# stephenbeckr/SparsifiedKMeans

Measured on AMD Instinct MI355X. Metric: Lloyd iters/sec + achieved HBM GB/s, N=1e8 d=1024 K=100, higher is better.
Workload: dtype f64

## Files before the change

### include/spkm.h

```cpp
#ifndef SPKM_H
#define SPKM_H
#include <stddef.h>
#include <stdint.h>

#ifdef __cplusplus
extern "C" {
#endif

#define SPKM_OK 0
#define SPKM_ERR_NULL_ARG (-1)
#define SPKM_ERR_CENTER_ROWS (-2)
#define SPKM_ERR_BETA_K (-3)
#define SPKM_ERR_LEN_LE_1 (-4)
#define SPKM_ERR_NOT_POW2 (-5)
#define SPKM_ERR_BAD_CSC (-6)
#define SPKM_ERR_UNSUPPORTED (-7)
#define SPKM_ERR_NO_DEVICE (-8)
#define SPKM_ERR_BAD_VALUE (-9)

typedef struct spkm_ctx spkm_ctx;
typedef struct spkm_shard spkm_shard;

const char *spkm_strerror(int status);
int spkm_version(void);

int spkm_ctx_create(int device, void *stream, spkm_ctx **out);
void spkm_ctx_destroy(spkm_ctx *ctx);
int spkm_ctx_sync(spkm_ctx *ctx);
int spkm_ctx_reload_switches(spkm_ctx *ctx);
int spkm_device_info(spkm_ctx *ctx, int64_t info[4]);


int spkm_SparseMatrixMinusCluster_host(spkm_ctx *ctx, uint64_t p, uint64_t n, const uint64_t *jc,
                                       const uint64_t *ir, const double *x, uint64_t c_rows, uint64_t K,
                                       const double *C, const double *beta, double *dist);

int spkm_SparseMatrixInnerProduct_host(spkm_ctx *ctx, uint64_t p, uint64_t n, const uint64_t *jc,
                                       const uint64_t *ir, const double *x, const double *c, double *ip,
                                       double *nx2);

int spkm_SparseMatrixColumnNormSq_host(spkm_ctx *ctx, uint64_t n, const uint64_t *jc, const double *x,
                                       double *nx2);

int spkm_hadamard_host(spkm_ctx *ctx, uint64_t m, uint64_t n, const double *x, double *y);
int spkm_hadamard_pthreads_host(spkm_ctx *ctx, uint64_t m, uint64_t n, const double *x, double *y);


int spkm_shard_create_host(spkm_ctx *ctx, uint64_t p, uint64_t n, const uint64_t *jc, const uint64_t *ir,
                           const double *x, spkm_shard **out);
int spkm_shard_create_dev(spkm_ctx *ctx, uint64_t p, uint64_t n, uint64_t nnz, const int64_t *d_jc,
                          const void *d_ir, int ir_bits, const double *d_x, uint64_t capacity,
                          spkm_shard **out);
int spkm_shard_reset_policy(spkm_shard *s);
int spkm_shard_set_lazy_stats(spkm_shard *s, int on);
int spkm_shard_set_wide_screen(spkm_shard *s, int on);
int spkm_shard_set_far_screen(spkm_shard *s, int on);
int spkm_shard_set_sliced_sums(spkm_shard *s, int on);
int spkm_shard_set_wide_bounds(spkm_shard *s, int on);
int spkm_shard_set_far_bounds(spkm_shard *s, int on);
int spkm_shard_set_far_events(spkm_shard *s, int on);
int spkm_shard_set_far_ragged(spkm_shard *s, int on);
int spkm_shard_set_tile_ragged(spkm_shard *s, int on);
int spkm_shard_release_csc(spkm_ctx *ctx, spkm_shard *s);
int spkm_shard_get_column_host(spkm_ctx *ctx, const spkm_shard *s, uint64_t col, uint64_t cap, uint64_t *ir_out,
                               double *x_out, uint64_t *count);
void spkm_shard_destroy(spkm_shard *s);
int spkm_shard_info(const spkm_shard *s, uint64_t *p, uint64_t *n, uint64_t *nnz, int *ir_bits);
int spkm_shard_order_info(const spkm_shard *s, int64_t info[2]);

uint64_t spkm_reduce_len(uint64_t p, uint64_t K);

int spkm_assign_dev(spkm_ctx *ctx, const spkm_shard *s, uint64_t K, const double *d_centers, double gamma,
                    int32_t *d_assign, double *d_mind, double *d_stats, uint64_t *d_nk_u64);

int spkm_assign_sparse_centers_dev(spkm_ctx *ctx, const spkm_shard *s, uint64_t K, const double *d_centers,
                                   const uint8_t *d_mask, double gamma, int32_t *d_assign, double *d_mind,
                                   double *d_stats, uint64_t *d_nk_u64);

int spkm_accumulate_dev(spkm_ctx *ctx, const spkm_shard *s, uint64_t K, const int32_t *d_assign,
                        double *d_reduce);

int spkm_assign_accumulate_dev(spkm_ctx *ctx, const spkm_shard *s, uint64_t K, const double *d_centers,
                               double gamma, int32_t *d_assign, double *d_mind, double *d_stats,
                               uint64_t *d_nk_u64, double *d_reduce);
int spkm_distances_dev(spkm_ctx *ctx, const spkm_shard *s, uint64_t K, const double *d_centers, double gamma,
                       const int32_t *d_assign, double *d_mind);
int spkm_distances_stats_dev(spkm_ctx *ctx, const spkm_shard *s, uint64_t K, const double *d_centers, double gamma,
                             const int32_t *d_assign, double *d_mind, double *d_stats);
int spkm_last_path_info(spkm_ctx *ctx, int64_t info[2]);
int spkm_last_screen_rounds(spkm_ctx *ctx, int64_t info[2]);
int spkm_last_screen_mode(spkm_ctx *ctx, int64_t info[8]);
int spkm_last_events_form(spkm_ctx *ctx, int64_t info[2]);
int spkm_last_assign_tile(spkm_ctx *ctx, int64_t info[6]);
int spkm_last_screen_tile(spkm_ctx *ctx, int64_t info[2]);
int spkm_last_screen_points(spkm_ctx *ctx, int64_t info[2]);
int spkm_last_mover_steps(spkm_ctx *ctx, uint64_t out[3]);
int spkm_last_mover_steps2(spkm_ctx *ctx, uint64_t out[3]);

int spkm_exact_pass_points(spkm_ctx *ctx, int64_t info[2]);
int spkm_screen_work_totals(spkm_ctx *ctx, int64_t info[2]);

int spkm_kpp_update_dev(spkm_ctx *ctx, uint64_t n, const double *d_dist_new, double *d_run, int first_round,
                        double *d_cum, double *total);
int spkm_kpp_draw_dev(spkm_ctx *ctx, uint64_t n, const double *d_cum, double target, int64_t *index);

int spkm_kpp_seed_dev(spkm_ctx *ctx, const spkm_shard *s, uint64_t K, double gamma, uint32_t R, const int64_t *first,
                      const double *u, int64_t *chosen, int32_t *status, double *d_run);
int spkm_last_kpp_plan(spkm_ctx *ctx, int info[4]);

int spkm_finalize_dev(spkm_ctx *ctx, uint64_t p, uint64_t K, const double *d_reduce, double gamma,
                      double *d_centers, double *d_out);

int spkm_fwht_dev(spkm_ctx *ctx, uint64_t m, uint64_t n, const double *d_x, double *d_y);
int spkm_mix_dev(spkm_ctx *ctx, uint64_t p, uint64_t p2, uint64_t n, const double *d_x, const double *d_sign,
                 double premul, double postdiv, double *d_y);

#define SPKM_MIX_MAX_P2 (1ull << 24)
#define SPKM_MIX_SCRATCH_BYTES (256ull << 20)
int spkm_mix_sample_dev(spkm_ctx *ctx, uint64_t p, uint64_t p2, uint64_t n, const double *d_x,
                        const double *d_sign, double premul, double postdiv, uint64_t s, uint64_t seed,
                        uint64_t col0, void *d_ir_out, int ir_bits, double *d_x_out);

uint64_t spkm_record_bytes(uint64_t s, int ir_bits);
int spkm_mix_sample_rec_dev(spkm_ctx *ctx, uint64_t p, uint64_t p2, uint64_t n, const double *d_x,
                            const double *d_sign, double premul, double postdiv, uint64_t s, uint64_t seed,
                            uint64_t col0, int ir_bits, void *d_rec_out);
#define SPKM_SKETCH_NONE 0
#define SPKM_SKETCH_DCT 1
int spkm_sketch_sample_dev(spkm_ctx *ctx, int kind, uint64_t p, uint64_t n, const double *d_x, const double *d_sign,
                           double premul, uint64_t s, uint64_t seed, uint64_t col0, void *d_ir_out, int ir_bits,
                           double *d_x_out);
int spkm_sketch_sample_rec_dev(spkm_ctx *ctx, int kind, uint64_t p, uint64_t n, const double *d_x, const double *d_sign,
                               double premul, uint64_t s, uint64_t seed, uint64_t col0, int ir_bits, void *d_rec_out);
#define SPKM_DCT_MAX_P 131072
int spkm_dct_sample_dev(spkm_ctx *ctx, uint64_t p, uint64_t n, const double *d_x, const double *d_sign, double premul,
                        uint64_t s, uint64_t seed, uint64_t col0, void *d_ir_out, int ir_bits, double *d_out);
int spkm_dct_sample_rec_dev(spkm_ctx *ctx, uint64_t p, uint64_t n, const double *d_x, const double *d_sign,
                            double premul, uint64_t s, uint64_t seed, uint64_t col0, int ir_bits, void *d_rec_out);
int spkm_dct_apply_dev(spkm_ctx *ctx, uint64_t p, uint64_t nvec, const double *d_in, const double *d_sign, int inverse,
                       double *d_out);
int spkm_shard_create_rec_dev(spkm_ctx *ctx, uint64_t p, uint64_t n, uint64_t s, int ir_bits, const void *d_rec,
                              spkm_shard **out);

#define SPKM_SRC_F64 0
#define SPKM_SRC_F32 1
#define SPKM_SRC_U8 2
#define SPKM_SRC_I16 3
#define SPKM_SRC_I32 4
#define SPKM_SRC_F16 5
#define SPKM_SRC_BF16 6
#define SPKM_SRC_I8 7
#define SPKM_SRC_U16 8

int spkm_widen_f64_dev(spkm_ctx *ctx, int kind, uint64_t count, const void *d_src, double *d_dst);

int spkm_mix_sample_src_dev(spkm_ctx *ctx, uint64_t p, uint64_t p2, uint64_t n, int src_kind, const void *d_src,
                            const double *d_sign, double premul, double postdiv, uint64_t s, uint64_t seed,
                            uint64_t col0, void *d_ir_out, int ir_bits, double *d_x_out);
int spkm_mix_sample_rec_src_dev(spkm_ctx *ctx, uint64_t p, uint64_t p2, uint64_t n, int src_kind, const void *d_src,
                                const double *d_sign, double premul, double postdiv, uint64_t s, uint64_t seed,
                                uint64_t col0, int ir_bits, void *d_rec_out);

int spkm_dense_assign_dev(spkm_ctx *ctx, uint64_t p, uint64_t n, const double *d_X, uint64_t K,
                          const double *d_centers, int32_t *d_assign, double *d_dist);
int spkm_dense_accumulate_dev(spkm_ctx *ctx, uint64_t p, uint64_t n, const double *d_X, uint64_t K,
                              const int32_t *d_assign, double *d_sums, double *d_counts);

int spkm_dense_assign_src_dev(spkm_ctx *ctx, uint64_t p, uint64_t n, int src_kind, const void *d_X, uint64_t K,
                              const double *d_centers, int32_t *d_assign, double *d_dist);
int spkm_dense_accumulate_src_dev(spkm_ctx *ctx, uint64_t p, uint64_t n, int src_kind, const void *d_X, uint64_t K,
                                  const int32_t *d_assign, double *d_sums, double *d_counts);

#define SPKM_COMM_ID_BYTES 128
#define SPKM_ERR_COMM (-10)

int spkm_comm_unique_id(uint8_t id[SPKM_COMM_ID_BYTES]);
int spkm_comm_init(spkm_ctx *ctx, int nranks, int rank, const uint8_t id[SPKM_COMM_ID_BYTES]);
int spkm_comm_destroy(spkm_ctx *ctx);
int spkm_comm_info(spkm_ctx *ctx, int *nranks, int *rank);
int spkm_allreduce_f64_dev(spkm_ctx *ctx, double *d_buf, uint64_t count);
// ... 19 lines not shown
```

### sparsifiedkmeans_amd/_lib.py

```python
from __future__ import annotations

import ctypes as C
import os
import re

_HERE = os.path.dirname(os.path.abspath(__file__))
_SO = os.path.join(_HERE, "libspkm.so")
HEADER = os.path.join(os.path.dirname(_HERE), "include", "spkm.h")

OK = 0
ERR_NULL_ARG, ERR_CENTER_ROWS, ERR_BETA_K, ERR_LEN_LE_1, ERR_NOT_POW2 = -1, -2, -3, -4, -5
ERR_BAD_CSC, ERR_UNSUPPORTED, ERR_NO_DEVICE, ERR_BAD_VALUE, ERR_COMM = -6, -7, -8, -9, -10
COMM_ID_BYTES = 128


class SpkmError(RuntimeError):

    def __init__(self, status: int, where: str = ""):
        self.status = status
        msg = lib().spkm_strerror(status).decode()
        super().__init__(f"{where + ': ' if where else ''}{msg} (spkm status {status})")


def _preload_hip_runtime() -> str:
# ... 33 lines not shown
_lib = None
hip_runtime_path = None

_u64 = C.c_uint64
_vp = C.c_void_p
_dbl = C.c_double


def declared_symbols() -> list[str]:
    with open(HEADER) as f:
        txt = f.read()
    return sorted(set(re.findall(r"\b(spkm_[A-Za-z0-9_]+)\s*\(", txt)))


def lib():
    global _lib, hip_runtime_path
    if _lib is not None:
        return _lib
    if not os.path.exists(_SO):
        raise ImportError(
            f"sparsifiedkmeans_amd: {_SO} is missing -- build it with "
            "`python -c 'import __graft_entry__ as g; g.build()'` or sparsifiedkmeans_amd/csrc/build.sh. "
            "There is no CPU fallback.")
    hip_runtime_path = _preload_hip_runtime()
    L = C.CDLL(_SO)
    L.spkm_strerror.restype = C.c_char_p
    L.spkm_strerror.argtypes = [C.c_int]
    L.spkm_version.restype = C.c_int
    L.spkm_ctx_create.argtypes = [C.c_int, _vp, C.POINTER(_vp)]
    L.spkm_ctx_destroy.argtypes = [_vp]
    L.spkm_ctx_destroy.restype = None
    L.spkm_ctx_sync.argtypes = [_vp]
    L.spkm_device_info.argtypes = [_vp, C.POINTER(C.c_int64)]
    L.spkm_SparseMatrixMinusCluster_host.argtypes = [_vp, _u64, _u64, _vp, _vp, _vp, _u64, _u64, _vp, _vp, _vp]
    L.spkm_SparseMatrixInnerProduct_host.argtypes = [_vp, _u64, _u64, _vp, _vp, _vp, _vp, _vp, _vp]
    L.spkm_SparseMatrixColumnNormSq_host.argtypes = [_vp, _u64, _vp, _vp, _vp]
    L.spkm_hadamard_host.argtypes = [_vp, _u64, _u64, _vp, _vp]
    L.spkm_hadamard_pthreads_host.argtypes = [_vp, _u64, _u64, _vp, _vp]
    L.spkm_shard_create_host.argtypes = [_vp, _u64, _u64, _vp, _vp, _vp, C.POINTER(_vp)]
    L.spkm_shard_create_dev.argtypes = [_vp, _u64, _u64, _u64, _vp, _vp, C.c_int, _vp, _u64, C.POINTER(_vp)]
    L.spkm_shard_destroy.argtypes = [_vp]
    L.spkm_shard_destroy.restype = None
    L.spkm_shard_info.argtypes = [_vp, C.POINTER(_u64), C.POINTER(_u64), C.POINTER(_u64), C.POINTER(C.c_int)]
    L.spkm_shard_order_info.argtypes = [_vp, C.POINTER(C.c_int64)]
    L.spkm_reduce_len.argtypes = [_u64, _u64]
    L.spkm_reduce_len.restype = _u64
    L.spkm_assign_dev.argtypes = [_vp, _vp, _u64, _vp, _dbl, _vp, _vp, _vp, _vp]
    L.spkm_assign_sparse_centers_dev.argtypes = [_vp, _vp, _u64, _vp, _vp, _dbl, _vp, _vp, _vp, _vp]
    L.spkm_accumulate_dev.argtypes = [_vp, _vp, _u64, _vp, _vp]
    L.spkm_assign_accumulate_dev.argtypes = [_vp, _vp, _u64, _vp, _dbl, _vp, _vp, _vp, _vp, _vp]
    L.spkm_last_path_info.argtypes = [_vp, C.POINTER(C.c_int64)]
    L.spkm_finalize_dev.argtypes = [_vp, _u64, _u64, _vp, _dbl, _vp, _vp]
    L.spkm_fwht_dev.argtypes = [_vp, _u64, _u64, _vp, _vp]
    L.spkm_mix_dev.argtypes = [_vp, _u64, _u64, _u64, _vp, _vp, _dbl, _dbl, _vp]
    L.spkm_mix_sample_dev.argtypes = [_vp, _u64, _u64, _u64, _vp, _vp, _dbl, _dbl, _u64, _u64, _u64, _vp, C.c_int, _vp]
    L.spkm_record_bytes.argtypes = [_u64, C.c_int]
    L.spkm_record_bytes.restype = _u64
    L.spkm_mix_sample_rec_dev.argtypes = [_vp, _u64, _u64, _u64, _vp, _vp, _dbl, _dbl, _u64, _u64, _u64, C.c_int, _vp]
    L.spkm_mix_sample_src_dev.argtypes = [_vp, _u64, _u64, _u64, C.c_int, _vp, _vp, _dbl, _dbl, _u64, _u64, _u64, _vp, C.c_int, _vp]
    L.spkm_mix_sample_rec_src_dev.argtypes = [_vp, _u64, _u64, _u64, C.c_int, _vp, _vp, _dbl, _dbl, _u64, _u64, _u64, C.c_int, _vp]
    L.spkm_sketch_sample_dev.argtypes = [_vp, C.c_int, _u64, _u64, _vp, _vp, _dbl, _u64, _u64, _u64, _vp, C.c_int, _vp]
    L.spkm_sketch_sample_rec_dev.argtypes = [_vp, C.c_int, _u64, _u64, _vp, _vp, _dbl, _u64, _u64, _u64, C.c_int, _vp]
    L.spkm_dct_sample_dev.argtypes = [_vp, _u64, _u64, _vp, _vp, _dbl, _u64, _u64, _u64, _vp, C.c_int, _vp]
    L.spkm_dct_sample_rec_dev.argtypes = [_vp, _u64, _u64, _vp, _vp, _dbl, _u64, _u64, _u64, C.c_int, _vp]
    L.spkm_dct_apply_dev.argtypes = [_vp, _u64, _u64, _vp, _vp, C.c_int, _vp]
    L.spkm_shard_create_rec_dev.argtypes = [_vp, _u64, _u64, _u64, C.c_int, _vp, C.POINTER(_vp)]
    L.spkm_last_screen_rounds.argtypes = [_vp, C.POINTER(C.c_int64)]
    L.spkm_last_screen_mode.argtypes = [_vp, C.POINTER(C.c_int64)]
    L.spkm_last_events_form.argtypes = [_vp, C.POINTER(C.c_int64)]
    L.spkm_last_assign_tile.argtypes = [_vp, C.POINTER(C.c_int64)]
    L.spkm_shard_reset_policy.argtypes = [_vp]
    L.spkm_shard_set_wide_screen.argtypes = [_vp, C.c_int]
    L.spkm_shard_set_wide_bounds.argtypes = [_vp, C.c_int]
    L.spkm_shard_set_far_screen.argtypes = [_vp, C.c_int]
    L.spkm_shard_set_far_bounds.argtypes = [_vp, C.c_int]
    L.spkm_shard_set_far_events.argtypes = [_vp, C.c_int]
    L.spkm_shard_set_far_ragged.argtypes = [_vp, C.c_int]
    L.spkm_shard_set_tile_ragged.argtypes = [_vp, C.c_int]
    L.spkm_shard_set_sliced_sums.argtypes = [_vp, C.c_int]
    L.spkm_last_screen_tile.argtypes = [_vp, C.POINTER(C.c_int64)]
    L.spkm_last_screen_points.argtypes = [_vp, C.POINTER(C.c_int64)]
    L.spkm_last_mover_steps.argtypes = [_vp, C.POINTER(C.c_uint64)]
    L.spkm_last_mover_steps2.argtypes = [_vp, C.POINTER(C.c_uint64)]
    L.spkm_dense_assign_dev.argtypes = [_vp, _u64, _u64, _vp, _u64, _vp, _vp, _vp]
    L.spkm_dense_accumulate_dev.argtypes = [_vp, _u64, _u64, _vp, _u64, _vp, _vp, _vp]
    L.spkm_dense_assign_src_dev.argtypes = [_vp, _u64, _u64, C.c_int, _vp, _u64, _vp, _vp, _vp]
    L.spkm_dense_accumulate_src_dev.argtypes = [_vp, _u64, _u64, C.c_int, _vp, _u64, _vp, _vp, _vp]
    L.spkm_last_assign_kernel_ms.argtypes = [_vp, C.POINTER(_dbl)]
    L.spkm_timing_log.argtypes = [_vp, C.c_int]
    L.spkm_timing_read.argtypes = [_vp, C.POINTER(_dbl), C.c_int, C.POINTER(C.c_int)]
    L.spkm_debug_block_times.argtypes = [_vp, C.c_int, C.POINTER(C.c_int64), C.c_int, C.POINTER(C.c_int)]
    L.spkm_debug_shard_bounds.argtypes = [_vp, _vp, _vp, _vp, _vp]
    L.spkm_exact_pass_points.argtypes = [_vp, C.POINTER(C.c_int64)]
    L.spkm_screen_work_totals.argtypes = [_vp, C.POINTER(C.c_int64)]
    L.spkm_distances_dev.argtypes = [_vp, _vp, _u64, _vp, _dbl, _vp, _vp]
    L.spkm_distances_stats_dev.argtypes = [_vp, _vp, _u64, _vp, _dbl, _vp, _vp, _vp]
    L.spkm_shard_set_lazy_stats.argtypes = [_vp, C.c_int]
    L.spkm_shard_release_csc.argtypes = [_vp, _vp]
    L.spkm_shard_get_column_host.argtypes = [_vp, _vp, _u64, _u64, _vp, _vp, C.POINTER(C.c_uint64)]
    L.spkm_kpp_update_dev.argtypes = [_vp, _u64, _vp, _vp, C.c_int, _vp, C.POINTER(C.c_double)]
    L.spkm_kpp_draw_dev.argtypes = [_vp, _u64, _vp, C.c_double, C.POINTER(C.c_int64)]
    L.spkm_kpp_seed_dev.argtypes = [_vp, _vp, _u64, C.c_double, C.c_uint32, _vp, _vp, _vp, _vp, _vp]
    L.spkm_last_kpp_plan.argtypes = [_vp, C.POINTER(C.c_int)]
    L.spkm_ctx_reload_switches.argtypes = [_vp]
    L.spkm_widen_f64_dev.argtypes = [_vp, C.c_int, _u64, _vp, _vp]
    L.spkm_comm_unique_id.argtypes = [_vp]
    L.spkm_comm_init.argtypes = [_vp, C.c_int, C.c_int, _vp]
    L.spkm_comm_destroy.argtypes = [_vp]
    L.spkm_comm_info.argtypes = [_vp, C.POINTER(C.c_int), C.POINTER(C.c_int)]
    L.spkm_allreduce_f64_dev.argtypes = [_vp, _vp, _u64]
    L.spkm_lloyd_iter.argtypes = [_vp, _vp, _u64, _vp, _dbl, C.c_int, _vp, _vp, _vp, _vp, _vp, _vp]
    L.spkm_lloyd_iter_host.argtypes = [_vp, _vp, _u64, _vp, _dbl, C.c_int, _vp, _vp, _vp, _vp, _vp, _vp, _vp]
    L.spkm_ctx_last_error.argtypes = [_vp]
    L.spkm_ctx_last_error.restype = C.c_char_p
    _lib = L
    return L


def check(status: int, where: str = ""):
    if status != 0:
        raise SpkmError(status, where)
```

### sparsifiedkmeans_amd/csrc/api.hip

```cpp
#include "fwht.hip"
#include "sparse_ops.hip"
#include "sample.hip"

#include "api_internal.h"
#include <chrono>
#include <sched.h>
#include <time.h>

static spkm_switches read_switches()
{
    auto on = [](const char* name) { const char* v = getenv(name); return v != nullptr && *v != 0 && !(v[0] == '0' && v[1] == 0); };
    spkm_switches w;
    w.no_screen = on("SPKM_NO_SCREEN");
    w.no_prune = on("SPKM_NO_PRUNE");
    w.no_hint = on("SPKM_NO_HINT");
    w.no_bounds = on("SPKM_NO_BOUNDS");
    w.no_rec = on("SPKM_NO_REC");
    w.no_point_list = on("SPKM_NO_POINT_LIST");
    w.no_cluster_skip = on("SPKM_NO_CLUSTER_SKIP");
    w.no_late_split = on("SPKM_NO_LATE_SPLIT");
    w.no_incremental = on("SPKM_NO_INCREMENTAL");
    w.no_support_drift = on("SPKM_NO_SUPPORT_DRIFT");
    w.no_teams = on("SPKM_NO_TEAMS");
    w.no_sums_only = on("SPKM_NO_SUMS_ONLY");
    w.no_dual = on("SPKM_NO_DUAL");
    w.no_block_skip = on("SPKM_NO_BLOCK_SKIP");
    w.no_direct_events = on("SPKM_NO_DIRECT_EVENTS");
    w.no_pair_events = on("SPKM_NO_PAIR_EVENTS");
    w.force_pair_events = on("SPKM_FORCE_PAIR_EVENTS");
    w.check_assign = on("SPKM_CHECK_ASSIGN");
    w.no_regroup = on("SPKM_NO_REGROUP");
    w.force_point_list = on("SPKM_FORCE_POINT_LIST");
    w.mover_tile = on("SPKM_NO_MOVER_TILE") ? -1 : (on("SPKM_MOVER_TILE") ? 1 : 0);
    w.mover_tile2 = on("SPKM_NO_MOVER_TILE2") ? -1 : (on("SPKM_MOVER_TILE2") ? 1 : 0);
    w.wide_screen = on("SPKM_WIDE_SCREEN");
    w.wide_bounds = on("SPKM_WIDE_BOUNDS");
    w.far_screen = on("SPKM_FAR_SCREEN");
    w.far_bounds = on("SPKM_FAR_BOUNDS");
    w.far_events = on("SPKM_FAR_EVENTS");
    w.far_ragged = on("SPKM_FAR_RAGGED");
    w.tile_ragged = on("SPKM_TILE_RAGGED");
    w.sliced_sums = on("SPKM_SLICED_SUMS");
    if (const char* v = getenv("SPKM_X_SLAB_ROWS")) w.x_slab_rows = std::max(0, atoi(v));
    if (const char* v = getenv("SPKM_FORCE_FORM")) w.force_form = std::max(0, std::min(3, atoi(v)));
    if (const char* v = getenv("SPKM_X_HINT_CHUNK")) w.x_hint_chunk = atoi(v);
    if (const char* v = getenv("SPKM_X_PLAIN_CHUNK")) w.x_plain_chunk = atoi(v);
    if (const char* v = getenv("SPKM_X_CERTIFY_GRID")) w.x_certify_grid = atoi(v);
    return w;
}

hipError_t allow_lds(spkm_ctx* ctx, const void* kern, size_t bytes)
{
    static std::mutex mu;
    static std::vector<std::tuple<int, const void*, size_t>> allowed;
    std::lock_guard<std::mutex> lock(mu);
    for (auto& e : allowed)
        if (std::get<0>(e) == ctx->device && std::get<1>(e) == kern) {
            if (std::get<2>(e) >= bytes) return hipSuccess;
            hipError_t r = hipFuncSetAttribute(kern, hipFuncAttributeMaxDynamicSharedMemorySize, (int)bytes);
            if (r == hipSuccess) std::get<2>(e) = bytes;
            return r;
        }
    hipError_t r = hipFuncSetAttribute(kern, hipFuncAttributeMaxDynamicSharedMemorySize, (int)bytes);
    if (r == hipSuccess) allowed.emplace_back(ctx->device, kern, bytes);
    return r;
}

int ensure(spkm_ctx* ctx, devbuf& b, size_t bytes)
{
    if (bytes <= b.cap && b.p) return SPKM_OK;
    if (b.p) ctx->sort_owner = nullptr;
    if (b.p) HIP_TRY(hipFree(b.p));
    b.p = nullptr;
    b.cap = 0;
    const size_t want = std::max<size_t>(bytes, 256);
    HIP_TRY(hipMalloc(&b.p, want));
    b.cap = want;
    return SPKM_OK;
}
void release(devbuf& b)
{
    if (b.p) (void)hipFree(b.p);
    b.p = nullptr;
    b.cap = 0;
}

extern "C" const char* spkm_strerror(int status)
{
    switch (status) {
    case SPKM_OK: return "ok";
    case SPKM_ERR_NULL_ARG: return "required pointer argument is NULL";
    case SPKM_ERR_CENTER_ROWS: return "Center vector must be or pxk, but this vector did not have p rows";
    case SPKM_ERR_BETA_K: return "Have not yet implemented case for using 'beta' with p x k (k!=1) centers";
    case SPKM_ERR_LEN_LE_1: return "Vector length must be greater than 1.";
    case SPKM_ERR_NOT_POW2: return "Vector length must be power of 2.";
    case SPKM_ERR_BAD_CSC: return "sparse matrix is not valid CSC (jc not monotone, row index out of range, or rows not ascending)";
    case SPKM_ERR_UNSUPPORTED: return "shape not supported by this build";
    case SPKM_ERR_NO_DEVICE: return "no usable HIP device (gfx950) available";
    case SPKM_ERR_BAD_VALUE: return "scalar argument out of range";
    case SPKM_ERR_COMM: return "RCCL is not available or an RCCL call failed (see spkm_ctx_last_error)";
    default: break;
    }
    if (status > 0) return hipGetErrorString((hipError_t)status);
    return "unknown spkm status";
}

extern "C" int spkm_version(void) { return SPKM_VERSION; }

extern "C" int spkm_ctx_create(int device, void* stream, spkm_ctx** out)
{
    if (!out) return SPKM_ERR_NULL_ARG;
    *out = nullptr;
    int ndev = 0;
    if (hipGetDeviceCount(&ndev) != hipSuccess || ndev <= 0 || device < 0 || device >= ndev)
        return SPKM_ERR_NO_DEVICE;
    spkm_ctx* ctx = new spkm_ctx();
    ctx->device = device;
    ctx->sw = read_switches();
    ctx->stream = (hipStream_t)stream;
    hipError_t e = hipSetDevice(device);
    hipDeviceProp_t prop;
    if (e == hipSuccess) e = hipGetDeviceProperties(&prop, device);
    if (e != hipSuccess) { delete ctx; return (int)e; }
    ctx->num_cus = prop.multiProcessorCount;
    ctx->mem_bytes = prop.totalGlobalMem;
    int lds = 0;
    if (hipDeviceGetAttribute(&lds, hipDeviceAttributeMaxSharedMemoryPerBlock, device) != hipSuccess || lds <= 0)
        lds = (int)prop.sharedMemPerBlock;
    ctx->lds_max = (size_t)lds;
    e = hipEventCreate(&ctx->ev0);
    if (e == hipSuccess) e = hipEventCreate(&ctx->ev1);
    if (e != hipSuccess) { delete ctx; return (int)e; }
    *out = ctx;
    return SPKM_OK;
}

extern "C" void spkm_ctx_destroy(spkm_ctx* ctx)
{
    if (!ctx) return;
    (void)hipSetDevice(ctx->device);
    (void)hipStreamSynchronize(ctx->stream);
    (void)spkm_comm_destroy(ctx);
    devbuf* all[] = {&ctx->tiles, &ctx->part_acc, &ctx->part_k, &ctx->blk_obj, &ctx->blk_max, &ctx->blk_imax,
                     &ctx->nk, &ctx->stats, &ctx->perm, &ctx->offs, &ctx->cursor, &ctx->items, &ctx->nitems,
                     &ctx->bmap, &ctx->blk_dff, &ctx->ct, &ctx->tmp_assign, &ctx->tmp_mind, &ctx->mscr, &ctx->dbg, &ctx->t32, &ctx->scr_m1, &ctx->scr_m2,
                     &ctx->scr_k, &ctx->cmax, &ctx->list, &ctx->nlist, &ctx->dn_x, &ctx->dn_c, &ctx->dn_nk, &ctx->bmapq, &ctx->bmapm, &ctx->bmapm2, &ctx->todo, &ctx->todo_m, &ctx->todo_m2, &ctx->bstat, &ctx->nk_ev, &ctx->fin_ticket, &ctx->wgstat, &ctx->offs2, &ctx->cursor2, &ctx->hist2,
                     &ctx->items2, &ctx->perm_o, &ctx->mix_scr};
    for (devbuf* b : all) release(*b);
    if (ctx->h_res) (void)hipHostFree(ctx->h_res);
    for (auto& pr : ctx->tlog) { (void)hipEventDestroy(pr.first); (void)hipEventDestroy(pr.second); }
    if (ctx->ev0) (void)hipEventDestroy(ctx->ev0);
    if (ctx->ev1) (void)hipEventDestroy(ctx->ev1);
    delete ctx;
}

extern "C" int spkm_ctx_reload_switches(spkm_ctx* ctx)
{
    if (!ctx) return SPKM_ERR_NULL_ARG;
    ctx->sw = read_switches();
    return SPKM_OK;
}

extern "C" int spkm_ctx_sync(spkm_ctx* ctx)
{
    if (!ctx) return SPKM_ERR_NULL_ARG;
    HIP_TRY(hipSetDevice(ctx->device));
    HIP_TRY(hipStreamSynchronize(ctx->stream));
    return SPKM_OK;
}

extern "C" int spkm_device_info(spkm_ctx* ctx, int64_t info[4])
{
    if (!ctx || !info) return SPKM_ERR_NULL_ARG;
    info[0] = ctx->num_cus;
    info[1] = (int64_t)ctx->lds_max;
    info[2] = (int64_t)ctx->mem_bytes;
    info[3] = SPKM_WAVE;
    return SPKM_OK;
}

static int validate_csc(uint64_t p, uint64_t n, const uint64_t* jc, const uint64_t* ir)
{
    if (jc[0] != 0) return SPKM_ERR_BAD_CSC;
    for (uint64_t i = 0; i < n; i++) {
        if (jc[i + 1] < jc[i]) return SPKM_ERR_BAD_CSC;
        for (uint64_t j = jc[i]; j < jc[i + 1]; j++) {
            if (ir[j] >= p) return SPKM_ERR_BAD_CSC;
            if (j > jc[i] && ir[j] <= ir[j - 1]) return SPKM_ERR_BAD_CSC;
        }
    }
    return SPKM_OK;
}

extern "C" int spkm_shard_create_host(spkm_ctx* ctx, uint64_t p, uint64_t n, const uint64_t* jc,
                                      const uint64_t* ir, const double* x, spkm_shard** out)
{
    if (!ctx || !out || !jc || (!ir && jc[n]) || (!x && jc[n])) return SPKM_ERR_NULL_ARG;
    *out = nullptr;
    if (p == 0 || p > 0x7fffffffull || n > 0x7ff00000ull) return SPKM_ERR_UNSUPPORTED;
    int rc = validate_csc(p, n, jc, ir);
    if (rc) return rc;
    HIP_TRY(hipSetDevice(ctx->device));
    const uint64_t nnz = jc[n];
    spkm_shard* s = new spkm_shard();
    s->ctx = ctx; s->p = p; s->n = n; s->nnz = nnz; s->owned = true; s->owned_csc = true;
    s->ir_bits = (p <= 65536) ? 16 : 32;
    s->slack = 48;
    if (n > 0 && nnz > 0 && nnz % n == 0) {
        const uint64_t st = nnz / n;
        bool fixed = st <= 0x7fffffffull;
        for (uint64_t i = 0; fixed && i <= n; i++) fixed = (jc[i] == i * st);
        if (fixed) s->fixed_s = (int)st;
    }
    {
        uint64_t mx = 0;
        for (uint64_t i = 0; i < n; i++) mx = std::max(mx, jc[i + 1] - jc[i]);
        s->max_s = (int)std::min<uint64_t>(mx, 0x7fffffffull);
        s->max_s_known = true;
    }
    const size_t irb = (size_t)s->ir_bits / 8;
    hipError_t e = hipMalloc((void**)&s->jc, (n + 1) * sizeof(long long));
    if (e == hipSuccess) e = hipMalloc(&s->ir, (nnz + 48) * irb);
    if (e == hipSuccess) e = hipMalloc((void**)&s->x, (nnz + 48) * sizeof(double));
    if (e == hipSuccess) e = hipMemsetAsync(s->ir, 0, (nnz + 48) * irb, ctx->stream);
    if (e == hipSuccess) e = hipMemsetAsync(s->x, 0, (nnz + 48) * sizeof(double), ctx->stream);
    if (e != hipSuccess) { spkm_shard_destroy(s); return (int)e; }
    std::vector<long long> jcn(n + 1);
    for (uint64_t i = 0; i <= n; i++) jcn[i] = (long long)jc[i];
    e = hipMemcpyAsync(s->jc, jcn.data(), (n + 1) * sizeof(long long), hipMemcpyHostToDevice, ctx->stream);
// ... 1060 lines not shown
```

### sparsifiedkmeans_amd/csrc/api_internal.h

```cpp
#pragma once
#include <hip/hip_runtime.h>

#include "../../include/spkm.h"
#include "layout.h"
#include "policy.h"

#include <dlfcn.h>

#include <algorithm>
#include <cmath>
#include <cstdio>
#include <cstdlib>
#include <cstring>
#include <utility>
#include <mutex>
#include <tuple>
#include <vector>

#define SPKM_VERSION 100

struct devbuf {
    void* p = nullptr;
    size_t cap = 0;
};

struct spkm_switches {
    bool no_screen = false;
    bool no_prune = false;
    bool no_hint = false;
    bool no_bounds = false;
    bool no_rec = false;
    bool no_point_list = false;
    bool no_cluster_skip = false;
    int x_hint_chunk = 0;
    int x_plain_chunk = 0;
    int x_certify_grid = 0;
    bool no_late_split = false;
    bool no_incremental = false;
    bool no_support_drift = false;
    bool no_sums_only = false;
    bool no_block_skip = false;
    bool no_dual = false;
    bool no_pair_events = false;
    bool force_pair_events = false;
    bool no_direct_events = false;
    bool no_teams = false;
    bool no_regroup = false;
    bool check_assign = false;
    int force_form = 0;
    bool wide_screen = false;
    bool wide_bounds = false;
    bool far_screen = false;
    bool far_bounds = false;
    bool far_events = false;
    bool far_ragged = false;
    bool tile_ragged = false;
    bool sliced_sums = false;
    int x_slab_rows = 0;
    bool force_point_list = false;
    int mover_tile2 = 0;
    int mover_tile = 0;
};
struct spkm_screen_report {
    int path = 0;
    int kt = 0, tiles = 0;
    int pl_last = 0;
    int rounds_all = 0, rounds = 0;
    int mode = 0;
    bool hinted = false;
    bool hint_late = false;
    bool skipping = false;
    bool pt_mode = false;
    bool lib_valid = false;
    bool incremental = false;
    bool direct_events = false;
    bool pair_events = false;
    bool sums_only = false;
    bool movers2 = false;
    bool movers = false;
    bool dual = false;
};
struct spkm_ctx {
    int device = 0;
    spkm_switches sw;
    hipStream_t stream = nullptr;
    int num_cus = 0;
    size_t lds_max = 0;
    size_t mem_bytes = 0;
    devbuf tiles, part_acc, part_k, blk_obj, blk_max, blk_imax, nk, stats, perm, offs, cursor, items, nitems,
        bmap, blk_dff, ct, tmp_assign, tmp_mind, mscr, dbg, t32, scr_m1, scr_m2, scr_k, cmax, list, nlist, dn_x, dn_c, dn_nk, bmapq, bmapm, bmapm2, todo, todo_m, todo_m2, bstat, nk_ev, fin_ticket, wgstat, offs2, cursor2, hist2, items2, perm_o;
    devbuf mix_scr;
    double* h_res = nullptr;
    double* h_res_dev = nullptr;
    size_t h_res_len = 0;
    unsigned long long res_seq = 0ull;
    bool res_map_failed = false;
    int bmap_G = -1, bmap_blocks = 0, bmap_streams = 0;
    int bmapq_key = -1, bmapq_blocks = 0;
    int bmapm_key = -1, bmapm_blocks = 0;
    int bmapm2_key = -1, bmapm2_blocks = 0;
    hipEvent_t ev0 = nullptr, ev1 = nullptr;
    bool ev_valid = false;
    std::vector<std::pair<hipEvent_t, hipEvent_t>> tlog;
    size_t tlog_used = 0;
    bool tlog_on = false;
    const void* sort_owner = nullptr;
    bool sort_partial = false;
    int sort_K = 0, sort_seg = 0;
    long long sort_n = 0;
    bool tlog_both = false;
    int assign_KT = 0, assign_G = 0;
    spkm_screen_report last;
    int last_exact_pts = 0;
    int last_acc_form = 0;
    int last_dist_form = 0;
    int last_kpp[4] = {0, 0, 0, 0};
    unsigned last_listed = 0;
    bool sort_perm_valid = false;
    char errmsg[256] = {0};
    void* comm = nullptr;
    int comm_nranks = 0, comm_rank = 0;
};

struct spkm_shard {
    spkm_ctx* ctx = nullptr;
    uint64_t p = 0, n = 0, nnz = 0;
    int ir_bits = 32;
    long long* jc = nullptr;
    void* ir = nullptr;
    double* x = nullptr;
    bool owned = false;
    bool owned_csc = false;
    int fixed_s = 0;
    uint64_t slack = 0;
    bool wide = false;
    bool wide_bounds = false;
    bool far = false;
    bool far_bounds = false;
    bool far_events = false;
    bool far_ragged = false;
    bool tile_ragged = false;
    int max_s = 0;
    bool max_s_known = false;
    bool sliced = false;
    float* xfs = nullptr;
    void* irs = nullptr;
    bool norms_done = false, xf_done = false;
    float* xnr = nullptr;
    float* xf = nullptr;
    char* rec = nullptr;
    int rec_R = 0;
    bool rec_owned = true;
    bool rec_tried = false;
    unsigned* h_nlist = nullptr;
    unsigned* h_nlist_dev = nullptr;
    unsigned nlist_seq = 0;
    bool nlist_pending = false;
    spkm_policy pol;
    float* hintu = nullptr;
    long long hintu_len = 0;
    float* hb = nullptr;
    double* hb_centers = nullptr;
    size_t hb_centers_len = 0;
    long long hb_npad = 0;
    int hb_K = 0;
    double hb_gamma = 0.0;
    bool hb_valid = false;
    char* sp = nullptr;
    long long sp_blocks = 0;
    bool sp_clean = false;
    const void* sp_assign = nullptr;
    bool assign_synced = false;
    double* hb_cum = nullptr;
// ... 37 lines not shown
```

### sparsifiedkmeans_amd/csrc/api_lloyd.hip

```cpp
#include "assign.hip"
#include "update.hip"
#include "kpp.hip"
#include "screen.hip"
#include "screen_wide.hip"
#include "screen_far.hip"
#include "dense.hip"

#include "api_internal.h"

const void* spkm_sq_kernel_16_0(int rounds, int a_rounds);
const void* spkm_sq_kernel_16_1(int rounds, int a_rounds);
const void* spkm_sq_kernel_32_0(int rounds, int a_rounds);
const void* spkm_sq_kernel_32_1(int rounds, int a_rounds);
template <typename IR> static const void* screen_quad_kernel(int rounds, int a_rounds, bool pts = false)
{
    if (sizeof(IR) == 2) return pts ? spkm_sq_kernel_16_1(rounds, a_rounds) : spkm_sq_kernel_16_0(rounds, a_rounds);
    return pts ? spkm_sq_kernel_32_1(rounds, a_rounds) : spkm_sq_kernel_32_0(rounds, a_rounds);
}

extern "C" int spkm_shard_create_rec_dev(spkm_ctx* ctx, uint64_t p, uint64_t n, uint64_t s_entries, int ir_bits,
                                         const void* d_rec, spkm_shard** out)
{
    if (!ctx || !out || (n && !d_rec)) return SPKM_ERR_NULL_ARG;
    *out = nullptr;
// ... 781 lines not shown
}

extern "C" int spkm_distances_dev(spkm_ctx* ctx, const spkm_shard* s, uint64_t K64, const double* d_centers, double gamma,
                                  const int32_t* d_assign, double* d_mind)
{
    return spkm_distances_stats_dev(ctx, s, K64, d_centers, gamma, d_assign, d_mind, nullptr);
}

extern "C" int spkm_exact_pass_points(spkm_ctx* ctx, int64_t info[2])
{
    if (!ctx || !info) return SPKM_ERR_NULL_ARG;
    info[0] = info[1] = 0;
    if (ctx->nlist.p) {
        HIP_TRY(hipSetDevice(ctx->device));
        HIP_TRY(hipStreamSynchronize(ctx->stream));
        unsigned v[NL_EXACT_TOTAL + 2] = {0};
        HIP_TRY(hipMemcpy(v, ctx->nlist.p, sizeof(v), hipMemcpyDeviceToHost));
        info[0] = (int64_t)(((unsigned long long)v[NL_EXACT_TOTAL + 1] << 32) | v[NL_EXACT_TOTAL]);
        info[1] = v[NL_EXACT_PTS];
    }
    return SPKM_OK;
}

extern "C" int spkm_screen_work_totals(spkm_ctx* ctx, int64_t info[2])
{
    if (!ctx || !info) return SPKM_ERR_NULL_ARG;
    info[0] = info[1] = 0;
    if (ctx->nlist.p) {
        HIP_TRY(hipSetDevice(ctx->device));
        HIP_TRY(hipStreamSynchronize(ctx->stream));
        static_assert(NL_ROUNDS_FULL == NL_ROUNDS_DONE + 2, "the two totals are copied together");
        unsigned long long v[2] = {0ull, 0ull};
        HIP_TRY(hipMemcpy(v, (const unsigned*)ctx->nlist.p + NL_ROUNDS_DONE, sizeof(v), hipMemcpyDeviceToHost));
        info[0] = (int64_t)v[0];
        info[1] = (int64_t)v[1];
    }
    return SPKM_OK;
}

extern "C" int spkm_last_screen_points(spkm_ctx* ctx, int64_t info[2])
{
    if (!ctx || !info) return SPKM_ERR_NULL_ARG;
    info[0] = info[1] = 0;
    if (ctx->nlist.p) {
        HIP_TRY(hipSetDevice(ctx->device));
        HIP_TRY(hipStreamSynchronize(ctx->stream));
        static_assert(NL_SCREENED == NL_SCREENED_TOTAL + 2, "the total and the call's count are copied together");
        unsigned v[3] = {0u, 0u, 0u};
        HIP_TRY(hipMemcpy(v, (const unsigned*)ctx->nlist.p + NL_SCREENED_TOTAL, sizeof(v), hipMemcpyDeviceToHost));
        info[1] = (int64_t)(((unsigned long long)v[1] << 32) | v[0]);
        info[0] = ctx->last.path == 1 ? (int64_t)v[2] : 0;
    }
    return SPKM_OK;
}

extern "C" int spkm_last_mover_steps(spkm_ctx* ctx, uint64_t out[3])
{
    if (!ctx || !out) return SPKM_ERR_NULL_ARG;
    out[0] = out[1] = out[2] = 0;
    if (ctx->last.path == 1 && ctx->nlist.p) {
        HIP_TRY(hipSetDevice(ctx->device));
        HIP_TRY(hipStreamSynchronize(ctx->stream));
        unsigned v[SPKM_REPORT_WORDS] = {0};
        HIP_TRY(hipMemcpy(v, ctx->nlist.p, sizeof(v), hipMemcpyDeviceToHost));
        out[0] = v[NL_MSTEPS]; out[1] = v[NL_MCERT]; out[2] = v[NL_MSENT];
    }
    return SPKM_OK;
}

extern "C" int spkm_last_mover_steps2(spkm_ctx* ctx, uint64_t out[3])
{
    if (!ctx || !out) return SPKM_ERR_NULL_ARG;
    out[0] = out[1] = out[2] = 0;
    if (ctx->last.path == 1 && ctx->nlist.p) {
        HIP_TRY(hipSetDevice(ctx->device));
        HIP_TRY(hipStreamSynchronize(ctx->stream));
        unsigned v[SPKM_REPORT_WORDS] = {0};
        HIP_TRY(hipMemcpy(v, ctx->nlist.p, sizeof(v), hipMemcpyDeviceToHost));
        out[0] = v[NL_MSTEPS2]; out[1] = v[NL_MCERT2]; out[2] = v[NL_MSENT2];
    }
    return SPKM_OK;
}

extern "C" int spkm_last_screen_rounds(spkm_ctx* ctx, int64_t info[2])
{
    if (!ctx || !info) return SPKM_ERR_NULL_ARG;
    info[0] = ctx->last.rounds_all;
    info[1] = ctx->last.rounds;
    return SPKM_OK;
}

extern "C" int spkm_last_screen_mode(spkm_ctx* ctx, int64_t info[8])
{
    if (!ctx || !info) return SPKM_ERR_NULL_ARG;
    info[0] = -1;
    info[1] = info[2] = info[3] = info[4] = info[5] = info[6] = info[7] = 0;
    const spkm_screen_report& r = ctx->last;
    if (r.path == 1 && ctx->nlist.p) {
        HIP_TRY(hipSetDevice(ctx->device));
        HIP_TRY(hipStreamSynchronize(ctx->stream));
        unsigned v[SPKM_REPORT_WORDS] = {0};
        HIP_TRY(hipMemcpy(v, ctx->nlist.p, sizeof(v), hipMemcpyDeviceToHost));
        info[0] = r.mode;
        info[1] = v[NL_LISTED]; info[2] = v[NL_AMBIG]; info[3] = v[NL_EARLY]; info[4] = v[NL_SKIPPED];
        info[5] = (int64_t)(((unsigned long long)v[NL_SKIPPED_TOTAL + 1] << 32) | v[NL_SKIPPED_TOTAL]);
        info[6] = r.incremental ? (r.direct_events ? 4 : 2) : (r.sums_only ? 3 : 0);
        if (r.dual) info[6] = v[NL_GATE_FULL] ? 3 : 2;
        info[7] = r.pt_mode ? 2 : 0;
    }
    return SPKM_OK;
}

extern "C" int spkm_last_events_form(spkm_ctx* ctx, int64_t info[2])
{
    if (!ctx || !info) return SPKM_ERR_NULL_ARG;
    const spkm_screen_report& r = ctx->last;
    info[0] = r.incremental ? (r.direct_events ? 2 : 1) : 0;
    info[1] = (r.incremental && r.pair_events) ? 1 : 0;
    return SPKM_OK;
}

extern "C" int spkm_last_assign_tile(spkm_ctx* ctx, int64_t info[6])
{
    if (!ctx || !info) return SPKM_ERR_NULL_ARG;
    info[0] = ctx->assign_KT;
    info[1] = ctx->assign_G;
    info[2] = ctx->last.pl_last;
    info[3] = ctx->last_exact_pts;
    info[4] = ctx->last_acc_form;
    info[5] = ctx->last_dist_form;
    return SPKM_OK;
}

extern "C" int spkm_last_screen_tile(spkm_ctx* ctx, int64_t info[2])
{
    if (!ctx || !info) return SPKM_ERR_NULL_ARG;
    info[0] = ctx->last.kt;
    info[1] = ctx->last.tiles;
    return SPKM_OK;
}

extern "C" int spkm_debug_shard_bounds(spkm_ctx* ctx, const spkm_shard* s, float* ub, double* lb, int32_t* lib_assign)
{
    if (!ctx || !s) return SPKM_ERR_NULL_ARG;
    if (!s->hb || !s->hb_valid || !s->hb_cum) return SPKM_ERR_UNSUPPORTED;
    HIP_TRY(hipSetDevice(ctx->device));
    HIP_TRY(hipStreamSynchronize(ctx->stream));
    const size_t n = (size_t)s->n, npad = (size_t)s->hb_npad;
    std::vector<int> map;
    if (s->map) {
        map.resize(n);
        HIP_TRY(hipMemcpy(map.data(), s->map, n * 4, hipMemcpyDeviceToHost));
    }
    auto at = [&](size_t i) { return s->map ? (size_t)map[i] : i; };
    std::vector<float> tmp(n);
    if (ub) {
        HIP_TRY(hipMemcpy(tmp.data(), s->hb, n * 4, hipMemcpyDeviceToHost));
        for (size_t i = 0; i < n; i++) ub[at(i)] = tmp[i];
    }
    if (lib_assign) {
        std::vector<int32_t> ta(n);
        HIP_TRY(hipMemcpy(ta.data(), s->hb + hb_assign(npad), n * 4, hipMemcpyDeviceToHost));
        for (size_t i = 0; i < n; i++) lib_assign[at(i)] = ta[i];
    }
    if (lb) {
        double cum = 0.0;
// ... 356 lines not shown
```

### sparsifiedkmeans_amd/csrc/api_lloyd_fused.inc

```
static int screen_tile_kt(const spkm_ctx* ctx, const spkm_shard* s)
{
    if ((s->p + 1) * (uint64_t)SCREEN_KT * 4 + 16 <= ctx->lds_max) return SCREEN_KT;
    return (s->wide || ctx->sw.wide_screen) ? spkm_wide_kt((long long)s->p, ctx->lds_max) : 0;
}
static bool screen_use_quad(const spkm_ctx* ctx, const spkm_shard* s)
{
    return spkm_screen_quad(screen_tile_kt(ctx, s), s->fixed_s);
}
static int screen_width(const spkm_ctx* ctx, const spkm_shard* s, int K)
{
    return spkm_screen_width((long long)s->p, K, s->fixed_s, s->slack, s->nnz, ctx->lds_max, ctx->num_cus, ctx->sw.no_screen,
                             s->wide || ctx->sw.wide_screen);
}
static int far_screen_width(const spkm_ctx* ctx, const spkm_shard* s, int K)
{
    if (s->fixed_s <= 0)
        return spkm_far_screen_ragged((long long)s->p, K, s->fixed_s, s->slack, s->nnz, ctx->lds_max, ctx->num_cus, ctx->sw.no_screen,
                                      s->far || ctx->sw.far_screen, s->far_ragged || ctx->sw.far_ragged);
    return spkm_far_screen((long long)s->p, K, s->fixed_s, s->slack, s->nnz, ctx->lds_max, ctx->num_cus, ctx->sw.no_screen,
                           s->wide || ctx->sw.wide_screen, s->far || ctx->sw.far_screen);
}
static int tile_ragged_width(const spkm_ctx* ctx, const spkm_shard* s, int K)
{
    return spkm_tile_screen_ragged((long long)s->p, K, s->fixed_s, s->slack, s->nnz, ctx->lds_max, ctx->num_cus, ctx->sw.no_screen,
                                   s->tile_ragged || ctx->sw.tile_ragged);
}

static_assert(spkm_movers == SPKM_MOVERS && spkm_movers == SCREEN_KT && spkm_mover_kmin == SPKM_MOVER_KMIN && spkm_mover_kmax == SPKM_MOVER_KMAX &&
              SPKM_MOVER_KMAX <= BOUNDS_KTAB, "the mover tile is one full screen tile; policy.h and layout.h agree on its limits");
static_assert(spkm_movers2 == SPKM_MOVERS2 && spkm_movers2 == 2 * SCREEN_KT && spkm_mover2_kmin == SPKM_MOVER2_KMIN,
              "the second level is two full screen tiles; policy.h and layout.h agree on its limits");
static_assert(spkm_plan_kt == SCREEN_KT && spkm_plan_span == BOUNDS_SPAN && spkm_plan_span_pt == BOUNDS_SPAN_PT &&
              spkm_plan_seg == SEG_POINTS, "policy.h sizes the kernels with these constants");

template <typename T>
static hipError_t regrow(T*& buf, size_t bytes, bool* valid = nullptr)
{
    if (buf) (void)hipFree(buf);
    buf = nullptr;
    if (valid) *valid = false;
    const hipError_t e = hipMalloc((void**)&buf, bytes);
    if (e != hipSuccess) buf = nullptr;
    return e;
}
static int ensure_blk_stats(spkm_ctx* ctx, size_t items)
{
    int rc;
    if ((rc = ensure(ctx, ctx->blk_obj, items * 8)) || (rc = ensure(ctx, ctx->blk_max, items * 8))) return rc;
    return ensure(ctx, ctx->blk_imax, items * 8);
}
static int count_assign_diff(spkm_ctx* ctx, const spkm_shard* s, const int32_t* d_assign, long long npad, unsigned* diff)
{
    const long long n = (long long)s->n;
    unsigned* cnt = (unsigned*)ctx->nlist.p + NL_CHECK_DIFF;
    HIP_TRY(hipMemsetAsync(cnt, 0, 4, ctx->stream));
    hipLaunchKernelGGL(k_count_diff_i32, dim3((unsigned)std::min<long long>(4096, (n + 255) / 256)), dim3(256), 0, ctx->stream,
                       (const int*)d_assign, (const int*)(s->hb + hb_assign(npad)), n, cnt, (const int*)s->map);
    HIP_TRY(hipMemcpyAsync(diff, cnt, 4, hipMemcpyDeviceToHost, ctx->stream));
    HIP_TRY(hipStreamSynchronize(ctx->stream));
    return SPKM_OK;
}
struct screen_call : spkm_call_in {
    spkm_ctx* ctx;
    spkm_shard* sm;
    const double* C;
    double gamma;
    int32_t* assign;
    double *mind, *sums, *counts;
    size_t pk;
    spkm_call_plan pl;
    spkm_mover_plan mv;
    spkm_mover2_plan mv2;
    spkm_screen_report rep;
    spkm_zero_jobs zj;
    int kt = SCREEN_KT;
    bool carry = false;
    int bstat_n = 0, seg = 0, max_items = 0;
    void zero_later(void* q, size_t bytes) { zj.p[zj.n] = (unsigned*)q; zj.words[zj.n] = bytes / 4; zj.n++; }
    void zero_flush()
    {
        if (!zj.n) return;
        unsigned long long mx = 0;
        for (int q = 0; q < zj.n; q++) mx = std::max(mx, zj.words[q]);
        hipLaunchKernelGGL(k_zero_many, dim3((unsigned)std::min<unsigned long long>((mx + 1023) / 1024, 256)), dim3(256), 0,
                           ctx->stream, zj);
        zj.n = 0;
    }
    int* cl(int row) const { return pl.cl_on ? sm->cl_flags + (size_t)row * K : nullptr; }
    int col_s() const { return sm->fixed_s > 0 ? sm->fixed_s : sm->max_s; }
    bool ragged() const { return sm->fixed_s <= 0; }
    template <typename IR> int buffers()
    {
        int rc;
        if (!quad && !sm->xnr) HIP_TRY(hipMalloc((void**)&sm->xnr, (size_t)n * 4));
        if (!quad && (rc = ensure_csc(ctx, sm))) return rc;
        if (!quad && !sm->xf) {
            HIP_TRY(hipMalloc((void**)&sm->xf, (size_t)(sm->nnz + 48) * 4));
            HIP_TRY(hipMemsetAsync(sm->xf, 0, (size_t)(sm->nnz + 48) * 4, ctx->stream));
        }
        if (!quad && (!sm->norms_done || !sm->xf_done)) {
            hipLaunchKernelGGL(k_point_norms, dim3((unsigned)std::min<long long>((n + 15) / 16, 16384)), dim3(256), 0,
                               ctx->stream, (const long long*)sm->jc, (const double*)sm->x, n, sm->fixed_s, sm->xnr, sm->xf);
            sm->norms_done = sm->xf_done = true;
        }
        if (quad && !sm->xfs) {
            if (!(sm->x == nullptr && sm->rec != nullptr) && (rc = ensure_csc(ctx, sm))) return rc;
            if ((rc = build_screen_copy<IR>(ctx, sm))) return rc;
        }
        const int Gs = pl.Gs;
        if (quad) rc = build_blockmap_quad(ctx, Gs, pl.pl_last, pl.nr);
        else rc = build_blockmap(ctx, pl.G);
        if (rc) return rc;
        if ((rc = ensure(ctx, ctx->t32, (size_t)(pl.G + (quad ? 2 : 0)) * (p + 1) * kt * 4)) || (rc = ensure(ctx, ctx->cmax, 64)) ||
            (rc = ensure(ctx, ctx->scr_m1, (size_t)Gs * n * 4)) || (rc = ensure(ctx, ctx->scr_m2, (size_t)Gs * n * 4)) ||
            (rc = ensure(ctx, ctx->scr_k, (size_t)Gs * n * 4)) || (rc = ensure(ctx, ctx->list, (size_t)n * 4)))
            return rc;
        {
            const bool fresh = ctx->nlist.p == nullptr;
            if ((rc = ensure(ctx, ctx->nlist, NL_WORDS * 4))) return rc;
            if (fresh) HIP_TRY(hipMemsetAsync(ctx->nlist.p, 0, NL_WORDS * 4, ctx->stream));
        }
        if ((rc = ensure(ctx, ctx->ct, pk * 8)) || (rc = ensure(ctx, ctx->nk, (size_t)K * 8)) || (rc = ensure(ctx, ctx->stats, 4 * 8)))
            return rc;
        zero_later(ctx->cmax.p, 16);
        zero_later((unsigned*)ctx->nlist.p + NL_ZERO_A, (NL_ZERO_A_END - NL_ZERO_A) * 4);
        zero_later((unsigned*)ctx->nlist.p + NL_ZERO_B, (NL_ZERO_B_END - NL_ZERO_B) * 4);
        zero_later(sums, (2 * pk + K + 1) * 8);
        if (!carry) return SPKM_OK;
        if (!sm->hb || sm->hb_npad != pl.npad) {
            HIP_TRY(regrow(sm->hb, hb_floats(pl.npad) * 4, &sm->hb_valid));
            sm->hb_npad = pl.npad;
            HIP_TRY(hipMemsetAsync(sm->hb + hb_mticket(pl.npad), 0, (size_t)(HB_TAIL - HB_MOVERS) * 4, ctx->stream));
        }
        if (sm->hb_centers_len < pk) {
            HIP_TRY(regrow(sm->hb_centers, pk * 8, &sm->hb_valid));
            sm->hb_centers_len = pk;
        }
        bounds_valid = sm->hb_valid && sm->hb_K == K && sm->hb_gamma == gamma;
        if (!sm->hb_cum) HIP_TRY(hipMalloc((void**)&sm->hb_cum, 16));
        if (quad && sm->pol.regroup_wanted && !sm->regroup_done && bounds_valid && sm->lazy && mind == nullptr && sm->rec != nullptr &&
            sm->xfs != nullptr && !ctx->sw.no_regroup) {
            if ((rc = regroup_shard<IR>(ctx, sm, K))) return rc;
            sm->regroup_done = true;
        }
        sm->pol.regroup_wanted = false;
        if (!bounds_valid) {
            HIP_TRY(hipMemsetAsync(sm->hb_cum, 0, 16, ctx->stream));
            sm->cum_par = 0;
        }
        if (far && far_events && sm->lazy) {
            if (!sm->cl_cache || sm->cl_pk != pk || sm->cl_K != K) {
                if (regrow(sm->cl_cache, cc_doubles(pk, K) * 8, &sm->cl_valid) != hipSuccess) {
                    (void)hipGetLastError();
                    sm->cl_pk = 0; sm->cl_K = 0;
                    far_events = false;
                } else {
                    sm->cl_pk = pk; sm->cl_K = K;
                }
            }
        }
        if (!quad) return SPKM_OK;
        if (!sm->cl_cache || sm->cl_pk != pk || sm->cl_K != K) {
            HIP_TRY(regrow(sm->cl_cache, cc_doubles(pk, K) * 8, &sm->cl_valid));
            HIP_TRY(regrow(sm->cl_flags, (size_t)CL_ROWS * K * 4));
            sm->cl_pk = pk; sm->cl_K = K;
        }
        zero_later(sm->cl_flags + (size_t)CL_TOUCHED * K, (size_t)K * 4);
        return SPKM_OK;
    }
    void plan_input(int prune_a_, bool want_hint_)
    {
        const spkm_switches& sw = ctx->sw;
        teams = quad ? ctx->bmapq_blocks / 4 : ctx->bmap_streams;
        no_bounds = sw.no_bounds; no_point_list = sw.no_point_list; force_point_list = sw.force_point_list;
        no_late_split = sw.no_late_split; no_incremental = sw.no_incremental; no_pair_events = sw.no_pair_events;
        force_pair_events = sw.force_pair_events; no_block_skip = sw.no_block_skip; no_cluster_skip = sw.no_cluster_skip;
        no_sums_only = sw.no_sums_only; no_dual = sw.no_dual; no_direct_events = sw.no_direct_events;
        x_hint_chunk = sw.x_hint_chunk; x_plain_chunk = sw.x_plain_chunk;
        lazy = sm->lazy; want_dist = mind != nullptr; has_map = sm->map != nullptr;
        cl_valid = sm->cl_valid; cl_stats_valid = sm->cl_stats_valid;
        sp_clean = sm->sp_clean; sp_blocks = sm->sp_blocks;
        same_assign = sm->sp_assign == (const void*)assign; assign_synced = sm->assign_synced;
        sort_kept = ctx->sort_owner == (const void*)sm && ctx->sort_K == K && ctx->sort_n == n;
        prune_a = prune_a_; want_hint = want_hint_;
    }
    int resources()
    {
        const size_t N = (size_t)n;
        if (pl.ev_possible && sm->ev_cap < 2 * N) {
            sm->ev_cap = 0;
            if (regrow(sm->ev_pt, 2 * N * 4 + 64) != hipSuccess || regrow(sm->ev_k, 2 * N * 4 + 64) != hipSuccess) {
                (void)hipGetLastError();
                pl.lose_events();
            } else
                sm->ev_cap = 2 * N;
        }
        if (pl.pair_ev && allow_lds(ctx, (const void*)k_plan_segments_wide, (size_t)K * (size_t)(K + 1) * 4) != hipSuccess) {
            (void)hipGetLastError();
            pl.lose_pair();
        }
        if (pl.pair_ev && sm->ev_o_cap < N + 4096) {
            sm->ev_o_cap = 0;
            if (regrow(sm->ev_o, (N + 4096) * 4 + 64) != hipSuccess) {
                (void)hipGetLastError();
                pl.lose_pair();
            } else
                sm->ev_o_cap = N + 4096;
        }
        int rc;
        if (pl.ev_path) {
            if ((rc = ensure(ctx, ctx->nk_ev, (size_t)2 * K * 8))) return rc;
            zero_later(ctx->nk_ev.p, (size_t)2 * K * 8);
        }
        if (pl.hinted) {
            rep.hint_late = pl.late;
            if (sm->hintu_len < pl.npad) {
                HIP_TRY(regrow(sm->hintu, (size_t)pl.npad * 4));
                sm->hintu_len = pl.npad;
            }
        }
        return SPKM_OK;
    }
    int mover_resources()
    {
        if (!mv.on) return SPKM_OK;
        int rc;
        if ((rc = build_blockmap_quad(ctx, mv.tiles, mv.pl, mv.nr, true))) return rc;
        if ((rc = ensure(ctx, ctx->todo_m, (size_t)mv.cap * 4))) return rc;
        if (!mv2.on) return SPKM_OK;
        if ((rc = build_blockmap_quad(ctx, mv2.tiles, mv2.pl, mv2.nr, true))) return rc;
        return ensure(ctx, ctx->todo_m2, (size_t)mv2.cap * 4);
    }
    int bounds()
    {
        const long long npad = pl.npad;
        if (!carry) {
            sm->hb_valid = sm->assign_synced = false;
            return SPKM_OK;
        }
        int* same = quad ? sm->cl_flags + (size_t)CL_SAME * K : (int*)nullptr;
        if (pl.drift) {
            zero_later(sm->hb + hb_dmax(npad, K), 4);
            zero_flush();
            hipLaunchKernelGGL(k_center_drift, dim3(K), dim3(256), 0, ctx->stream, (const double*)sm->hb_centers, C, K, p,
                               gamma, sm->hb + hb_delta(npad), same, ctx->sw.no_support_drift ? 0 : col_s(),
                               2.0f * (float)sm->fixed_s / (float)p, quad ? sm->hb + hb_hterm(npad) : (float*)nullptr,
                               mv.eligible ? reinterpret_cast<unsigned*>(sm->hb + hb_mticket(npad)) : (unsigned*)nullptr,
                               sm->hb + hb_mdr(npad), reinterpret_cast<int*>(sm->hb + hb_mlist(npad)),
                               reinterpret_cast<int*>(sm->hb + hb_mslot(npad)));
            int rc;
            if ((rc = ensure(ctx, ctx->todo, pl.pt_mode ? (size_t)(npad + 64) * 4 : (size_t)(npad / 16 + 1) * 4))) return rc;
            if ((rc = ensure(ctx, ctx->bstat, (size_t)pl.bgrid * BS_STRIDE * 4))) return rc;
            const long long nblk = npad / 1024 + 1;
            if (pl.sp_on && sm->sp_blocks != nblk) {
                HIP_TRY(regrow(sm->sp, sp_bytes(nblk), &sm->sp_clean));
                sm->sp_blocks = nblk;
            }
            unsigned* sp_mask = pl.sp_on ? reinterpret_cast<unsigned*>(sm->sp) : nullptr;
            float* sp_slack = pl.sp_on ? reinterpret_cast<float*>(sm->sp + sp_off_slack(nblk)) : nullptr;
            int* sp_valid = pl.sp_on ? reinterpret_cast<int*>(sm->sp + sp_off_valid(nblk)) : nullptr;
            if (((pl.sp_on && !pl.sp_reset) || pl.trusted) && ctx->sw.check_assign) {
                unsigned diff = 0;
                if ((rc = count_assign_diff(ctx, sm, assign, npad, &diff))) return rc;
                if (diff) {
                    snprintf(ctx->errmsg, sizeof(ctx->errmsg), "SPKM_CHECK_ASSIGN: d_assign differs from the library's copy of the previous "
                             "call's assignment in %u places (lazy statistics: the buffer is the library's to keep between calls)", diff);
                    sm->sp_clean = false;
                    sm->assign_synced = false;
                    return SPKM_ERR_BAD_VALUE;
                }
            }
            const long long blocks = std::min<long long>((npad + pl.span - 1) / pl.span, pl.bgrid);
            hipLaunchKernelGGL(sm->map != nullptr ? k_bounds_steps<true> : (mv.eligible ? k_bounds_steps<false, true> : k_bounds_steps<false>),
                               dim3((unsigned)blocks), dim3(256), 0,
                               ctx->stream, sm->hb, npad, n, K, pl.trusted ? (int*)nullptr : (int*)assign, (int*)ctx->todo.p,
                               (unsigned*)ctx->nlist.p, pl.hinted ? sm->hintu : (float*)nullptr, pl.skip_enabled ? 1 : 0,
                               pl.pt_mode ? 1 : 0, (const double*)(sm->hb_cum + sm->cum_par), sm->hb_cum + (sm->cum_par ^ 1),
                               (int)pl.span, (unsigned*)ctx->bstat.p, pl.erode ? 1 : 0, sp_slack, sp_mask, sp_valid, pl.sp_reset ? 1 : 0,
                               (const int*)same, (const int*)sm->map, mv.on ? (int*)ctx->todo_m.p : (int*)nullptr,
                               mv2.on ? (int*)ctx->todo_m2.p : (int*)nullptr);
            bstat_n = (int)blocks;
            if (pl.skip_enabled) sm->cum_par ^= 1;
        }
        sm->sp_clean = pl.drift && pl.sp_on;
        sm->sp_assign = (const void*)assign;
        sm->assign_synced = true;
        sm->hb_valid = false;
        return SPKM_OK;
    }
    template <typename IR> int screen()
    {
        zero_flush();
        const size_t tile_floats = (size_t)pl.G * (p + 1) * kt;
        if (kt == SCREEN_KT)
            hipLaunchKernelGGL(k_prep_tiles_f32, dim3((unsigned)std::min<size_t>((tile_floats + 255) / 256, 2048)), dim3(256),
                               0, ctx->stream, C, p, K, pl.G, gamma, (float*)ctx->t32.p,
                               (unsigned long long*)ctx->cmax.p, pl.pl_last, quad ? 1 : 0, (double*)ctx->ct.p,
                               carry ? sm->hb_centers : (double*)nullptr,
                               mv.on ? reinterpret_cast<const int*>(sm->hb + hb_mlist(pl.npad)) : (const int*)nullptr, mv2.on ? 2 : 1);
        else
            hipLaunchKernelGGL(k_prep_tiles_wide, dim3((unsigned)std::min<size_t>((tile_floats + 255) / 256, 2048)), dim3(256),
                               0, ctx->stream, C, p, K, pl.G, kt, gamma, (float*)ctx->t32.p,
                               (unsigned long long*)ctx->cmax.p, (double*)ctx->ct.p, carry ? sm->hb_centers : (double*)nullptr);
        rep.pl_last = pl.pl_last;
        rep.kt = kt;
        rep.tiles = pl.Gs;
        const size_t lds = (size_t)(p + 1) * (kt * 4 + (pl.pl_last == 5 ? 16 : 0)) + 16;
        const bool wlist = !quad && pl.skip_enabled;
        const void* kern = quad ? screen_quad_kernel<IR>(pl.nr, pl.prune_a > 0 ? pl.prune_a : pl.nr, pl.pt_mode)
                           : wlist ? (kt == SCREEN_KT ? (const void*)k_screen_wide<IR, 32, true>
                                                      : (kt == 16 ? (const void*)k_screen_wide<IR, 16, true> : (const void*)k_screen_wide<IR, 8, true>))
                                   : (kt == SCREEN_KT ? (const void*)k_screen_tile<IR>
                                                      : (kt == 16 ? (const void*)k_screen_wide<IR, 16> : (const void*)k_screen_wide<IR, 8>));
        HIP_TRY(allow_lds(ctx, kern, lds));
        HIP_TRY(timing_begin(ctx));
        const IR* a_ir = quad ? (const IR*)sm->irs : (const IR*)sm->ir;
        const float* a_xf = quad ? (const float*)sm->xfs : (const float*)sm->xf;
        const float* a_t = (const float*)ctx->t32.p;
        int a_p = p, a_n = (int)n, a_s = sm->fixed_s, a_K = K, a_chunk = (int)pl.chunk;
        const spkm_blockmap* a_bm = (const spkm_blockmap*)(quad ? ctx->bmapq.p : ctx->bmap.p);
        float *a_m1 = (float*)ctx->scr_m1.p, *a_m2 = (float*)ctx->scr_m2.p;
        int* a_k = (int*)ctx->scr_k.p;
        int a_extra = pl.G - 1;
        rep.rounds_all = quad ? pl.rounds_all : 0;
        rep.rounds = quad ? pl.nr : 0;
        const float* a_hint = (pl.hinted && pl.rounds_all < pl.nr) ? sm->hintu : nullptr;
        float a_hc = 1.5f;
        rep.hinted = a_hint != nullptr;
        rep.mode = rep.hinted ? 2 : (rep.rounds_all < rep.rounds ? 1 : 0);
        unsigned* a_cnt = (unsigned*)ctx->nlist.p;
        const int* a_todo = pl.skip_enabled ? (const int*)ctx->todo.p : nullptr;
        const char* a_rec = (pl.pt_mode && sm->rec) ? sm->rec : (const char*)nullptr;
        int a_recR = sm->rec_R, a_tp = pl.pt_mode ? 1 : 0;
        const int* a_recmap = sm->map;
        int a_slot = NL_TODO;
        void* args[] = {&a_ir, &a_xf, &a_t, &a_p, &a_n, &a_s, &a_K, &a_bm, &a_chunk, &a_m1, &a_m2, &a_k, &a_extra,
                        &a_hint, &a_hc, &a_cnt, &a_todo, &a_tp, &a_rec, &a_recR, &a_recmap, &a_slot};
        if (mv.on) {
            const float* m_t = a_t + (size_t)pl.G * (p + 1) * SCREEN_KT;
            const spkm_blockmap* m_bm = (const spkm_blockmap*)ctx->bmapm.p;
            const int* m_todo = (const int*)ctx->todo_m.p;
            int m_K = SPKM_MOVERS, m_extra = 0, m_slot = NL_TODO_M;
            void* margs[] = {&a_ir, &a_xf, &m_t, &a_p, &a_n, &a_s, &m_K, &m_bm, &a_chunk, &a_m1, &a_m2, &a_k, &m_extra,
                             &a_hint, &a_hc, &a_cnt, &m_todo, &a_tp, &a_rec, &a_recR, &a_recmap, &m_slot};
            HIP_TRY(hipLaunchKernel(kern, dim3(ctx->bmapm_blocks), dim3(1024), margs, lds, ctx->stream));
            HIP_TRY(hipGetLastError());
            const int* m2_todo = (const int*)ctx->todo_m2.p;
            if (mv2.on) {
                const spkm_blockmap* m2_bm = (const spkm_blockmap*)ctx->bmapm2.p;
                int m2_K = SPKM_MOVERS2, m2_slot = NL_TODO_M2;
                void* m2args[] = {&a_ir, &a_xf, &m_t, &a_p, &a_n, &a_s, &m2_K, &m2_bm, &a_chunk, &a_m1, &a_m2, &a_k, &m_extra,
                                  &a_hint, &a_hc, &a_cnt, &m2_todo, &a_tp, &a_rec, &a_recR, &a_recmap, &m2_slot};
                HIP_TRY(hipLaunchKernel(kern, dim3(ctx->bmapm2_blocks), dim3(1024), m2args, lds, ctx->stream));
                HIP_TRY(hipGetLastError());
            }
            hipLaunchKernelGGL(k_certify_movers<1>, dim3((unsigned)std::min<long long>(4096, (n + 1023) / 1024)), dim3(256), 0, ctx->stream,
                               (const float*)ctx->scr_m1.p, (const float*)ctx->scr_m2.p, (const int*)ctx->scr_k.p, n, (const float*)sm->xnr,
                               col_s(), (const unsigned long long*)ctx->cmax.p, sm->hb, pl.npad, K, m_todo, (int*)ctx->todo.p,
                               (unsigned*)ctx->nlist.p, (const double*)(sm->hb_cum + (sm->cum_par ^ 1)), (const double*)(sm->hb_cum + sm->cum_par));
            HIP_TRY(hipGetLastError());
            if (mv2.on) {
                hipLaunchKernelGGL(k_certify_movers<2>, dim3((unsigned)std::min<long long>(4096, (n + 1023) / 1024)), dim3(256), 0, ctx->stream,
                                   (const float*)ctx->scr_m1.p, (const float*)ctx->scr_m2.p, (const int*)ctx->scr_k.p, n, (const float*)sm->xnr,
                                   col_s(), (const unsigned long long*)ctx->cmax.p, sm->hb, pl.npad, K, m2_todo, (int*)ctx->todo.p,
                                   (unsigned*)ctx->nlist.p, (const double*)(sm->hb_cum + (sm->cum_par ^ 1)), (const double*)(sm->hb_cum + sm->cum_par));
                HIP_TRY(hipGetLastError());
            }
        }
        rep.movers = mv.on;
        rep.movers2 = mv2.on;
        const long long* a_jc = nullptr;
        void* args_w[] = {&a_ir, &a_xf, &a_t, &a_p, &a_n, &a_s, &a_K, &a_bm, &a_chunk, &a_m1, &a_m2, &a_k, &a_todo, &a_cnt, &a_jc};
        const bool wide_args = !quad && (wlist || kt != SCREEN_KT);
        HIP_TRY(hipLaunchKernel(kern, dim3(quad ? ctx->bmapq_blocks : ctx->bmap_blocks), dim3(1024), wide_args ? args_w : args, lds,
                                ctx->stream));
        HIP_TRY(hipGetLastError());
        HIP_TRY(timing_end(ctx));
        rep.skipping = pl.skip_enabled;
        rep.pt_mode = pl.pt_mode;
        return SPKM_OK;
    }
    template <typename IR> int screen_far()
    {
        zero_flush();
        const size_t tile_floats = (size_t)pl.G * (p + 1) * kt;
        hipLaunchKernelGGL(k_prep_tiles_wide, dim3((unsigned)std::min<size_t>((tile_floats + 255) / 256, 2048)), dim3(256), 0,
                           ctx->stream, C, p, K, pl.G, kt, gamma, (float*)ctx->t32.p, (unsigned long long*)ctx->cmax.p,
                           (double*)ctx->ct.p, carry ? sm->hb_centers : (double*)nullptr);
        rep.pl_last = pl.pl_last;
        rep.kt = kt;
        rep.tiles = pl.Gs;
        rep.rounds_all = rep.rounds = 0;
        rep.mode = 0;
        const int npl = kt / 64;
        const bool flist = pl.skip_enabled;
        const void* kern = flist ? (npl == 1 ? (const void*)k_screen_far<IR, 1, true>
                                             : (npl == 2 ? (const void*)k_screen_far<IR, 2, true> : (const void*)k_screen_far<IR, 4, true>))
                                 : (npl == 1 ? (const void*)k_screen_far<IR, 1> : (npl == 2 ? (const void*)k_screen_far<IR, 2> : (const void*)k_screen_far<IR, 4>));
        if (ragged())
            kern = flist ? (npl == 1 ? (const void*)k_screen_far<IR, 1, true, true>
                                     : (npl == 2 ? (const void*)k_screen_far<IR, 2, true, true> : (const void*)k_screen_far<IR, 4, true, true>))
                         : (npl == 1 ? (const void*)k_screen_far<IR, 1, false, true>
                                     : (npl == 2 ? (const void*)k_screen_far<IR, 2, false, true> : (const void*)k_screen_far<IR, 4, false, true>));
        HIP_TRY(timing_begin(ctx));
        const IR* a_ir = (const IR*)sm->ir;
        const float* a_xf = (const float*)sm->xf;
        const float* a_t = (const float*)ctx->t32.p;
        int a_p = p, a_n = (int)n, a_s = sm->fixed_s, a_K = K;
        float *a_m1 = (float*)ctx->scr_m1.p, *a_m2 = (float*)ctx->scr_m2.p;
        int* a_k = (int*)ctx->scr_k.p;
        const int* a_todo = flist ? (const int*)ctx->todo.p : (const int*)nullptr;
        const unsigned* a_cnt = (const unsigned*)ctx->nlist.p;
        const long long* a_jc = (const long long*)sm->jc;
        void* args[] = {&a_ir, &a_xf, &a_t, &a_p, &a_n, &a_s, &a_K, &a_m1, &a_m2, &a_k, &a_todo, &a_cnt, &a_jc};
        const unsigned gx = (unsigned)std::min<long long>((n + 3) / 4, (long long)std::max(1, num_cus) * 32);
        HIP_TRY(hipLaunchKernel(kern, dim3(gx, (unsigned)pl.G), dim3(256), args, 0, ctx->stream));
        HIP_TRY(hipGetLastError());
        HIP_TRY(timing_end(ctx));
        rep.skipping = pl.skip_enabled;
        rep.pt_mode = pl.pt_mode;
        return SPKM_OK;
    }
    template <typename IR> int screen_tile_ragged()
    {
        zero_flush();
        const size_t tile_floats = (size_t)pl.G * (p + 1) * kt;
        hipLaunchKernelGGL(k_prep_tiles_wide, dim3((unsigned)std::min<size_t>((tile_floats + 255) / 256, 2048)), dim3(256), 0,
                           ctx->stream, C, p, K, pl.G, kt, gamma, (float*)ctx->t32.p, (unsigned long long*)ctx->cmax.p,
                           (double*)ctx->ct.p, carry ? sm->hb_centers : (double*)nullptr);
        rep.pl_last = pl.pl_last;
        rep.kt = kt;
        rep.tiles = pl.Gs;
        rep.rounds_all = rep.rounds = 0;
        rep.mode = 0;
        const bool wlist = pl.skip_enabled;
// ... 266 lines not shown
            hipLaunchKernelGGL(k_zero_u64_gated, dim3((K + 255) / 256), dim3(256), 0, ctx->stream,
                               (unsigned long long*)ctx->nk.p, K, gate);
            hipLaunchKernelGGL(k_hist, dim3((unsigned)std::min<long long>(1024, (n + 1023) / 1024)), dim3(256), (size_t)K * 4,
                               ctx->stream, (const int*)assign, n, K, (unsigned long long*)ctx->nk.p, gate);
        }
        if (pl.cl_on)
            hipLaunchKernelGGL(k_cluster_need, dim3(1), dim3(256), 0, ctx->stream, cl(CL_TOUCHED), (const int*)cl(CL_SAME),
                               pl.cl_skip ? 0 : 1, K, (const unsigned long long*)ctx->nk.p, cl(CL_NEED), (unsigned*)ctx->nlist.p);
        hipLaunchKernelGGL(k_plan_segments, dim3(1), dim3(256), 0, ctx->stream, (const unsigned long long*)ctx->nk.p, K,
                           seg, (long long*)ctx->offs.p, (unsigned long long*)ctx->cursor.p, (int4*)ctx->items.p,
                           (int*)ctx->nitems.p, pl.cl_on ? (const unsigned*)nullptr : gate, (const int*)cl(CL_NEED), cl(CL_IBEG), cl(CL_ICNT));
        int sb = (int)std::max<long long>(std::min<long long>(1024, (n + 1023) / 1024), std::min<long long>(8192, n / 4096));
        const size_t sc_lds = (size_t)((K + 1) & ~1) * 4 + (size_t)K * 12;
        launch_scatter(ctx, sb, sc_lds, (const int*)assign, n, K, pl.cl_on ? (const unsigned*)nullptr : gate,
                       pl.cl_skip ? (const int*)cl(CL_NEED) : (const int*)nullptr);
        ctx->sort_partial = pl.cl_skip;
        if (quad) {
            ctx->sort_owner = sm; ctx->sort_K = K; ctx->sort_n = n; ctx->sort_seg = seg;
            ctx->sort_perm_valid = true;
        }
        const int threads = 1024, nw = threads / 64;
        const size_t per_pt = (size_t)(sm->fixed_s | 1) * 8;
        const size_t fixed_lds = (size_t)p * 20 + 16;
        int pts = (int)std::min<size_t>(64, (ctx->lds_max - fixed_lds - 1024) / nw / per_pt);
        pts = std::max(8, pts & ~7);
        const size_t lds2 = fixed_lds + (size_t)nw * pts * per_pt;
        const void* k2 = pl.use_rec ? (const void*)k_exact_accumulate<IR, 16, 4, false, true> : (const void*)k_exact_accumulate<IR, 16, 4, false, false>;
        HIP_TRY(allow_lds(ctx, (const void*)k2, lds2));
        const int ab = std::min(max_items, std::max(1, ctx->num_cus));
        int rc;
        if ((rc = ensure_blk_stats(ctx, (size_t)std::max(ab, max_items)))) return rc;
        if (ctx->tlog_both) HIP_TRY(timing_begin(ctx));
        float* ub = (carry && sm->map == nullptr) ? sm->hb : (float*)nullptr;
        ctx->last_exact_pts = pl.pipe ? 16 : pts;
        if (pl.pipe) {
            if ((rc = exact_rec<IR>(!pl.sums_only, mind, ub, ab))) return rc;
        } else {
            hipLaunchKernelGGL((pl.use_rec ? k_exact_accumulate<IR, 16, 4, false, true> : k_exact_accumulate<IR, 16, 4, false, false>),
                               dim3(ab), dim3(threads), lds2, ctx->stream, (const char*)sm->rec, sm->rec_R, (const IR*)sm->ir,
                               (const double*)sm->x, (const int*)ctx->perm.p, (const long long*)ctx->offs.p, (const int4*)ctx->items.p,
                               (const int*)ctx->nitems.p, C, gamma, p, sm->fixed_s, pts, mind, ub, sums, counts,
                               (double*)ctx->blk_obj.p, (double*)ctx->blk_max.p, (long long*)ctx->blk_imax.p);
        }
        if (ctx->tlog_both) HIP_TRY(timing_end(ctx));
        if (pl.cl_on) {
            double *cache_s = sm->cl_cache, *cache_c = cache_s + cc_counts(pk), *cl_obj = cache_s + cc_obj(pk), *cl_max = cache_s + cc_max(pk, K);
            long long* cl_imax = reinterpret_cast<long long*>(cache_s + cc_imax(pk, K));
            hipLaunchKernelGGL(k_cluster_restore, dim3((unsigned)std::min<size_t>((pk + 255) / 256, 2048)), dim3(256), 0, ctx->stream,
                               (const int*)cl(CL_TOUCHED) , K, p, sums, counts, cache_s, cache_c);
            if (!pl.sums_only)
                hipLaunchKernelGGL(k_cluster_stats, dim3(1), dim3(256), 0, ctx->stream, (const int*)cl(CL_NEED), K, (const int*)cl(CL_IBEG),
                                   (const int*)cl(CL_ICNT), (const double*)ctx->blk_obj.p, (const double*)ctx->blk_max.p,
                                   (const long long*)ctx->blk_imax.p, cl_obj, cl_max, cl_imax, (double*)ctx->stats.p);
            sm->cl_valid = true;
            sm->cl_stats_valid = !pl.sums_only;
        } else {
            sm->cl_valid = false;
            sm->cl_stats_valid = false;
            if (pl.pipe) {
                hipLaunchKernelGGL(k_reduce_stats_n, dim3(1), dim3(64), 0, ctx->stream, (const double*)ctx->blk_obj.p,
                                   (const double*)ctx->blk_max.p, (const long long*)ctx->blk_imax.p, (const int*)ctx->nitems.p,
                                   (double*)ctx->stats.p);
            } else
                hipLaunchKernelGGL(k_reduce_stats, dim3(1), dim3(64), 0, ctx->stream, (const double*)ctx->blk_obj.p,
                                   (const double*)ctx->blk_max.p, (const long long*)ctx->blk_imax.p, ab, (double*)ctx->stats.p);
        }
        return SPKM_OK;
    }
    int tail(double* d_stats, uint64_t* d_nk_u64, bool no_stats = false)
    {
        const bool ev = pl.ev_path;
        double* nk_f = sums + 2 * pk;
        const unsigned long long work_steps = (unsigned long long)((n + 15) / 16);
        const int work_tiles = quad ? pl.Gs : 0;
        const int work_flags = ((quad && rep.rounds_all < rep.rounds && !rep.hinted) ? 1 : 0) |
                               (pl.skip_enabled ? 2 : 0) | (pl.pt_mode ? 4 : 0);
        const unsigned grid = ev ? (unsigned)std::max<size_t>((K + 255) / 256, std::min<size_t>((pk + 255) / 256, 1024)) : (unsigned)(K + 255) / 256;
        hipLaunchKernelGGL(k_call_tail, dim3(grid), dim3(256), 0, ctx->stream, (const unsigned long long*)ctx->nk.p, K, nk_f,
                           (const double*)ctx->stats.p, nk_f + K, d_stats, (unsigned long long*)d_nk_u64, (const unsigned*)ctx->bstat.p,
                           bstat_n, (unsigned*)ctx->nlist.p, (ev || pl.sums_only || no_stats) ? 1 : 0, ev ? sm->cl_cache : (double*)nullptr,
                           ev ? (const double*)(sm->cl_cache + cc_counts(pk)) : (const double*)nullptr, ev ? pk : (size_t)0,
                           ev ? sums : (double*)nullptr, ev ? counts : (double*)nullptr,
                           sm->nlist_pending ? (unsigned*)nullptr : sm->h_nlist_dev, sm->nlist_seq + 1u,
                           work_steps, work_tiles, pl.nr, rep.rounds_all, work_flags, (unsigned long long)n, (mv.on ? 1 : 0) | (mv2.on ? 2 : 0));
        HIP_TRY(hipGetLastError());
        if (carry) {
            sm->hb_K = K; sm->hb_gamma = gamma; sm->hb_valid = true;
        }
        if (ev) {
            sm->cl_stats_valid = false;
            ctx->sort_owner = sm;
            ctx->sort_K = K; ctx->sort_n = n; ctx->sort_perm_valid = false; ctx->sort_partial = false;
        }
        rep.path = 1;
        return SPKM_OK;
    }
};

template <typename IR>
static int run_screen(spkm_ctx* ctx, const spkm_shard* s, int K, const double* d_centers, double gamma,
                      int32_t* d_assign, double* d_mind, double* d_reduce, int prune_a, bool want_hint,
                      double* d_stats, uint64_t* d_nk_u64, int kt, spkm_screen_report* report)
{
    screen_call c;
    c.kt = kt;
    c.ctx = ctx; c.sm = const_cast<spkm_shard*>(s); c.C = d_centers; c.gamma = gamma; c.assign = d_assign; c.mind = d_mind;
    c.n = (long long)s->n; c.p = (int)s->p; c.K = K; c.fixed_s = c.max_s = s->fixed_s; c.quad = spkm_screen_quad(kt, s->fixed_s);
    c.carry_bounds = !c.quad && (s->wide_bounds || ctx->sw.wide_bounds); c.carry = c.quad || c.carry_bounds;
    c.lds_max = ctx->lds_max; c.num_cus = ctx->num_cus; c.pk = (size_t)c.p * K; c.sums = d_reduce; c.counts = d_reduce + c.pk;
    c.zj.n = 0;
    c.seg = seg_points(c.n, ctx->num_cus); c.max_items = (int)(c.n / c.seg) + K + 1;
    spkm_plan_tiles(c.pl, c, kt);
    int rc;
    if ((rc = c.buffers<IR>())) return rc;
    c.plan_input(prune_a, want_hint);
    spkm_plan_call(c.pl, c, c.sm->pol);
    c.mv = spkm_plan_movers(c, c.pl, K, ctx->sw.mover_tile);
    c.mv2 = spkm_plan_movers2(c.mv, c.pl, K, ctx->sw.mover_tile2);
    if ((rc = c.resources()) || (rc = c.mover_resources()) || (rc = c.bounds()) || (rc = c.screen<IR>())) return rc;
    const int ev = c.pl.ev_possible ? 2 : 1, max_items_ev_all = ev == 2 ? (int)((2 * c.n) / SEG_EVENTS) + 2 * K + 1 : 0;
    if ((rc = ensure(ctx, ctx->perm, (size_t)ev * c.n * 4)) || (rc = ensure(ctx, ctx->offs, (size_t)(ev * K + 1) * 8)) ||
        (rc = ensure(ctx, ctx->cursor, (size_t)ev * K * 8)) ||
        (rc = ensure(ctx, ctx->items, (size_t)std::max(c.max_items, max_items_ev_all) * 16)) || (rc = ensure(ctx, ctx->nitems, NI_WORDS * 4)))
        return rc;
    if ((rc = build_records<IR>(ctx, c.sm))) return rc;
    if (!c.sm->rec && (rc = ensure_csc(ctx, s))) return rc;
    c.sort_reusable = ctx->sort_owner == (const void*)s && ctx->sort_perm_valid && ctx->sort_seg == c.seg && !ctx->sort_partial;
    spkm_plan_sums(c.pl, c, c.sm->pol, c.sm->rec != nullptr);
    c.rep.sums_only = c.pl.sums_only;
    c.rep.dual = c.pl.dual;
    if ((rc = c.certify<IR>()) || (rc = c.pl.ev_path ? c.events<IR>() : c.full_pass<IR>())) return rc;
    if ((rc = c.tail(d_stats, d_nk_u64))) return rc;
    *report = c.rep;
    return SPKM_OK;
}

template <typename IR>
static int run_far(spkm_ctx* ctx, const spkm_shard* s, int K, const double* d_centers, double gamma, int32_t* d_assign,
                   double* d_mind, double* d_reduce, double* d_stats, uint64_t* d_nk_u64, int kp, spkm_screen_report* report,
                   bool tile = false)
{
    screen_call c;
    c.kt = kp;
    c.ctx = ctx; c.sm = const_cast<spkm_shard*>(s); c.C = d_centers; c.gamma = gamma; c.assign = d_assign; c.mind = d_mind;
    c.n = (long long)s->n; c.p = (int)s->p; c.K = K; c.fixed_s = s->fixed_s; c.quad = false; c.far = true;
    c.carry_bounds = c.carry = s->far_bounds || ctx->sw.far_bounds;
    c.far_events = c.carry && (s->far_events || ctx->sw.far_events);
    c.lds_max = ctx->lds_max; c.num_cus = ctx->num_cus; c.pk = (size_t)c.p * K; c.sums = d_reduce; c.counts = d_reduce + c.pk;
    c.zj.n = 0;
    int rc;
    if ((rc = ensure_max_s(ctx, c.sm))) return rc;
    c.max_s = c.sm->max_s;
    spkm_plan_tiles(c.pl, c, kp);
    if ((rc = c.buffers<IR>())) return rc;
    c.plan_input(0, false);
    spkm_plan_call(c.pl, c, c.sm->pol);
    const spkm_acc_plan ap = spkm_accumulate_form((long long)s->p, ctx->lds_max, s->sliced || ctx->sw.sliced_sums, ctx->sw.x_slab_rows);
    if (c.pl.ev_path && !c.pl.direct && ap.form == 2) c.pl.lose_events();
    if ((rc = c.resources()) || (rc = c.bounds()) || (rc = tile ? c.screen_tile_ragged<IR>() : c.screen_far<IR>()) ||
        (rc = c.certify<IR>()))
        return rc;
    bool no_stats = c.pl.ev_path;
    if ((rc = c.pl.ev_path ? c.far_events_apply<IR>(ap) : c.far_sums(&no_stats)) || (rc = c.tail(d_stats, d_nk_u64, no_stats))) return rc;
    *report = c.rep;
    return SPKM_OK;
}

extern "C" int spkm_assign_accumulate_dev(spkm_ctx* ctx, const spkm_shard* s, uint64_t K64, const double* d_centers,
                                          double gamma, int32_t* d_assign, double* d_mind, double* d_stats,
                                          uint64_t* d_nk_u64, double* d_reduce)
{
    if (!ctx || !s || !d_centers || !d_assign || !d_reduce) return SPKM_ERR_NULL_ARG;
    if (K64 == 0 || K64 > 65536) return SPKM_ERR_UNSUPPORTED;
    HIP_TRY(hipSetDevice(ctx->device));
    int rc;
    spkm_shard* sm = const_cast<spkm_shard*>(s);
    if (!sm->h_nlist) {
        HIP_TRY(hipHostMalloc((void**)&sm->h_nlist, SPKM_REPORT_BUF_WORDS * 4, hipHostMallocMapped | hipHostMallocCoherent));
        memset(sm->h_nlist, 0, SPKM_REPORT_BUF_WORDS * 4);
        HIP_TRY(hipHostGetDevicePointer((void**)&sm->h_nlist_dev, sm->h_nlist, 0));
    }
    if (sm->nlist_pending && __atomic_load_n(sm->h_nlist + SPKM_REPORT_WORDS, __ATOMIC_ACQUIRE) == sm->nlist_seq) {
        sm->nlist_pending = false;
        const unsigned* h = sm->h_nlist;
        ctx->last_listed = h[NL_LISTED];
        spkm_policy_counters c;
        c.listed = h[NL_LISTED]; c.ambig = h[NL_AMBIG]; c.early = h[NL_EARLY]; c.skipped = h[NL_SKIPPED];
        c.kept = h[NL_KEPT]; c.movers = h[NL_MOVERS];
        c.msteps = (double)h[NL_MCERT] + (double)h[NL_MCERT2];
        c.pairs2 = 2.0 * ((double)h[NL_MCERT2] + (double)h[NL_MSENT2]);
        c.early2 = h[NL_MEARLY2];
        c.full_opened = h[NL_GATE_FULL] != 0u;
        c.one_cluster_steps = h[NL_ONE_CLUSTER];
        c.may_regroup = sm->pend_full && sm->lazy && !sm->regroup_done;
        const int kt_seen = std::max(8, screen_tile_kt(ctx, s));
        sm->pol.observe(c, (double)s->n, (int)((K64 + kt_seen - 1) / kt_seen), (s->fixed_s + 3) / 4);
    }
    spkm_policy::choice ch = sm->pol.next(ctx->sw.no_prune, ctx->sw.no_hint, screen_use_quad(ctx, s));
    if (ctx->sw.force_form) {
        ch.exact = false;
        ch.prune_a = ctx->sw.force_form == 2 ? 1 : 0;
        ch.want_hint = ctx->sw.force_form == 3 && screen_use_quad(ctx, s);
    }
    const bool cooling = ch.exact;
    const int kt = screen_width(ctx, s, (int)K64);
    int kp = kt > 0 ? 0 : far_screen_width(ctx, s, (int)K64);
    const bool tile_ragged = kt == 0 && kp == 0 && (kp = tile_ragged_width(ctx, s, (int)K64)) > 0;
    if (s->n > 0 && !cooling && (kt > 0 || kp > 0)) {
        ctx->ev_valid = false;
        const int prune_a = ch.prune_a;
        const bool want_hint = ch.want_hint;
        spkm_screen_report rep;
        if (kp > 0)
            rc = (s->ir_bits == 16) ? run_far<unsigned short>(ctx, s, (int)K64, d_centers, gamma, d_assign, d_mind, d_reduce, d_stats, d_nk_u64, kp, &rep, tile_ragged)
                                    : run_far<unsigned int>(ctx, s, (int)K64, d_centers, gamma, d_assign, d_mind, d_reduce, d_stats, d_nk_u64, kp, &rep, tile_ragged);
        else
            rc = (s->ir_bits == 16) ? run_screen<unsigned short>(ctx, s, (int)K64, d_centers, gamma, d_assign, d_mind, d_reduce, prune_a, want_hint, d_stats, d_nk_u64, kt, &rep)
                                    : run_screen<unsigned int>(ctx, s, (int)K64, d_centers, gamma, d_assign, d_mind, d_reduce, prune_a, want_hint, d_stats, d_nk_u64, kt, &rep);
        if (rc) return rc;
        ctx->last = rep;
        if (!sm->nlist_pending) {
            sm->nlist_seq++;
            sm->nlist_pending = true;
            sm->pol.launched(rep.rounds_all, rep.rounds, rep.hinted, rep.hint_late, rep.skipping, rep.lib_valid, rep.incremental, rep.dual);
            sm->pend_full = kp == 0 && !rep.skipping && screen_use_quad(ctx, s);
        }
        return SPKM_OK;
    }
    ctx->last = spkm_screen_report();
    sm->sp_clean = false;
    sm->assign_synced = false;
    sm->hb_valid = false;
    if (!d_mind) {
        if ((rc = ensure(ctx, ctx->mscr, (size_t)std::max<uint64_t>(s->n, 1) * 8))) return rc;
        d_mind = (double*)ctx->mscr.p;
    }
    rc = spkm_assign_dev(ctx, s, K64, d_centers, gamma, d_assign, d_mind, d_stats, d_nk_u64);
    if (rc) return rc;
    return spkm_accumulate_dev(ctx, s, K64, d_assign, d_reduce);
}
```

### sparsifiedkmeans_amd/csrc/layout.h

```cpp
#pragma once
#include <cstddef>

enum spkm_counter_slot : int {
    NL_LISTED = 0,
    NL_AMBIG = 1,
    NL_EARLY = 2,
    NL_SKIPPED = 3,
    NL_TODO = 4,
    NL_CHANGED = 5,
    NL_MSTEPS = 6,
    NL_TODO_M = 7,
    NL_SKIPPED_TOTAL = 8,
    NL_MCERT = 10,
    NL_MSENT = 11,
    NL_KEPT = 12,
    NL_EXACT_PTS = 13,
    NL_MOVERS = 14,
    NL_EVENTS = 16,
    NL_GATE_EVENTS = 18,
    NL_GATE_FULL = 19,
    NL_CHECK_DIFF = 20,
    NL_ONE_CLUSTER = 21,
    NL_MEARLY = 22,
    NL_MSTEPS2 = 23,
    NL_TODO_M2 = 24,
    NL_MCERT2 = 25,
    NL_MSENT2 = 26,
    NL_MEARLY2 = 27,
    NL_PER_CALL_END = 32,
    NL_EXACT_TOTAL = 32,
    NL_ROUNDS_DONE = 34,
    NL_ROUNDS_FULL = 36,
    NL_SCREENED_TOTAL = 38,
    NL_SCREENED = 40,
    NL_WORDS = 64
};
constexpr int SPKM_REPORT_WORDS = 28;
constexpr int SPKM_REPORT_BUF_WORDS = 32;
constexpr int NL_ZERO_A = 0, NL_ZERO_A_END = NL_SKIPPED_TOTAL;
constexpr int NL_ZERO_B = NL_SKIPPED_TOTAL + 2, NL_ZERO_B_END = NL_PER_CALL_END;

constexpr bool nl_zeroed(int w) { return (w >= NL_ZERO_A && w < NL_ZERO_A_END) || (w >= NL_ZERO_B && w < NL_ZERO_B_END); }
constexpr bool nl_reported(int w) { return w < SPKM_REPORT_WORDS; }
constexpr bool nl_total_ok(int w) { return w % 2 == 0 && w + 1 < NL_WORDS && !nl_zeroed(w) && !nl_zeroed(w + 1); }
static_assert(nl_reported(NL_LISTED) && nl_reported(NL_AMBIG) && nl_reported(NL_EARLY) && nl_reported(NL_SKIPPED) &&
              nl_reported(NL_KEPT) && nl_reported(NL_MOVERS) && nl_reported(NL_GATE_FULL) && nl_reported(NL_ONE_CLUSTER),
              "every counter the host policy reads is in the report");
static_assert(SPKM_REPORT_WORDS + 1 <= SPKM_REPORT_BUF_WORDS && SPKM_REPORT_WORDS <= NL_WORDS, "the report and its number fit");
static_assert(NL_SCREENED < NL_WORDS && NL_ONE_CLUSTER < NL_PER_CALL_END, "every slot fits the buffer");
static_assert(nl_reported(NL_MSTEPS) && nl_reported(NL_MCERT) && nl_reported(NL_MSENT) && nl_zeroed(NL_MSTEPS) && nl_zeroed(NL_TODO_M) &&
              nl_zeroed(NL_MCERT) && nl_zeroed(NL_MSENT) && nl_zeroed(NL_MEARLY) && NL_MEARLY < SPKM_REPORT_WORDS,
              "the mover tile's counters are per-call words of the report");
static_assert(nl_reported(NL_MSTEPS2) && nl_reported(NL_MCERT2) && nl_reported(NL_MSENT2) && nl_reported(NL_MEARLY2) && nl_zeroed(NL_MSTEPS2) &&
              nl_zeroed(NL_TODO_M2) && nl_zeroed(NL_MCERT2) && nl_zeroed(NL_MSENT2) && nl_zeroed(NL_MEARLY2),
              "... and so are the second level's");
static_assert(nl_total_ok(NL_SKIPPED_TOTAL) && nl_total_ok(NL_EXACT_TOTAL) && nl_total_ok(NL_ROUNDS_DONE) &&
              nl_total_ok(NL_ROUNDS_FULL) && nl_total_ok(NL_SCREENED_TOTAL),
              "a running total is an aligned 64-bit pair that the per-call zeroing leaves alone");
static_assert(!nl_zeroed(NL_SCREENED) && nl_zeroed(NL_EXACT_PTS) && nl_zeroed(NL_GATE_FULL), "per-call words are zeroed, NL_SCREENED is not");

enum { WG_AMBIG = 0, WG_CHANGED = 1, WG_MOVERS = 2, WG_ONE_CLUSTER = 3, WG_STRIDE = 4 };
enum { BS_KEPT = 0, BS_SKIPPED = 1, BS_STRIDE = 2 };
enum { NI_FULL = 0, NI_EVENTS = 1, NI_PAIR_CHUNKS = 2, NI_REGROUP = 4, NI_WORDS = 16 };

constexpr int HB_KMAX = 65536;
constexpr int HB_HTERM = HB_KMAX + 16;
constexpr int SPKM_MOVERS = 32;
constexpr int SPKM_MOVERS2 = 64;
constexpr int SPKM_MOVER_KMIN = 64, SPKM_MOVER_KMAX = 1024;
constexpr int SPKM_MOVER2_KMIN = 96;
constexpr int HB_MOVERS = 2 * HB_KMAX + 32;
constexpr int HB_MTICKET = HB_MOVERS, HB_MDR = HB_MOVERS + 1, HB_MLIST = HB_MOVERS + 16, HB_MDR2 = HB_MDR + 1, HB_MSLOT = HB_MLIST + SPKM_MOVERS2;
constexpr int HB_TAIL = HB_MSLOT + SPKM_MOVER_KMAX + 16;
static_assert(HB_HTERM + HB_KMAX <= HB_MOVERS && HB_MLIST % 4 == 0, "the movers lie behind hterm[], the list 16-byte aligned");
static_assert(HB_MDR2 < HB_MLIST && HB_MLIST + SPKM_MOVERS2 <= HB_MSLOT && SPKM_MOVERS2 == 2 * SPKM_MOVERS,
              "both drifts lie in front of the list, the list of two tiles in front of the slots");
constexpr long long hb_lb(long long npad) { return npad; }
constexpr long long hb_assign(long long npad) { return 2 * npad; }
constexpr long long hb_delta(long long npad) { return 3 * npad; }
constexpr long long hb_dmax(long long npad, int K) { return 3 * npad + K; }
constexpr long long hb_hterm(long long npad) { return 3 * npad + HB_HTERM; }
constexpr long long hb_mticket(long long npad) { return 3 * npad + HB_MTICKET; }
constexpr long long hb_mdr(long long npad) { return 3 * npad + HB_MDR; }
constexpr long long hb_mdr2(long long npad) { return 3 * npad + HB_MDR2; }
constexpr long long hb_mlist(long long npad) { return 3 * npad + HB_MLIST; }
constexpr long long hb_mslot(long long npad) { return 3 * npad + HB_MSLOT; }
constexpr size_t hb_floats(long long npad) { return (size_t)3 * npad + HB_TAIL; }

constexpr int SP_MASK_WORDS = 4;
constexpr size_t sp_off_slack(size_t nblk) { return nblk * SP_MASK_WORDS * 4; }
constexpr size_t sp_off_valid(size_t nblk) { return nblk * (SP_MASK_WORDS * 4 + 4); }
constexpr size_t sp_bytes(size_t nblk) { return nblk * (SP_MASK_WORDS * 4 + 8); }

constexpr size_t cc_counts(size_t pk) { return pk; }
constexpr size_t cc_obj(size_t pk) { return 2 * pk; }
constexpr size_t cc_max(size_t pk, size_t K) { return 2 * pk + K; }
constexpr size_t cc_imax(size_t pk, size_t K) { return 2 * pk + 2 * K; }
constexpr size_t cc_doubles(size_t pk, size_t K) { return 2 * pk + 3 * K; }
enum { CL_NEED = 0, CL_TOUCHED = 1, CL_SAME = 2, CL_IBEG = 3, CL_ICNT = 4, CL_ROWS = 5 };
```

### sparsifiedkmeans_amd/csrc/policy.h

```cpp
#pragma once
#include <algorithm>
#include <cmath>

#ifdef __HIPCC__
#define SPKM_HD __host__ __device__
#else
#define SPKM_HD
#endif

SPKM_HD constexpr int quad_split_late(int nr, bool pts = false)
{
    return pts ? (nr >= 10 ? (nr + 1) / 2 : 0) : (nr >= 6 ? ((nr + 2) / 4 > 2 ? (nr + 2) / 4 : 2) : 0);
}
SPKM_HD constexpr int quad_split(int nr, bool pts = false)
{
    return nr < 3 ? nr : (pts ? ((nr + 2) / 4 > 2 ? (nr + 2) / 4 : 2) : (nr / 8 > 1 ? nr / 8 : 1));
}

struct spkm_policy_counters {
    double listed = 0, ambig = 0, early = 0, skipped = 0, kept = 0, movers = 0;
    double msteps = 0;
    double pairs2 = 0, early2 = 0;
    bool full_opened = false;
    double one_cluster_steps = 0;
    bool may_regroup = false;
};

struct spkm_policy {
    int prune_pending_a = 0;
    bool hint_pending = false;
    bool hint_late_pending = false;
    bool skip_pending = false;
    bool mov_pending_valid = false;
    bool ev_latched = false;
    bool dual_latched = false;
    int exact_cooldown = 0;
    int prune_next_a = 0;
    int prune_cooldown = 0;
    bool hint_late = true;
    int hint_late_left = 3;
    int hint_cooldown = 0;
    int hint_fail_streak = 0;
    bool pt_next = false;
    bool blocks_next = false;
    bool crowded = false;
    bool regroup_wanted = false;
    bool movers_known = false;
    unsigned long long last_movers = 0;
    bool ev_pending = false;
    int ev_calls = 0;
    unsigned long long ev_cum_movers = 0;

    static constexpr unsigned long long direct_events_below = 2048;
    bool events_direct() const { return movers_known && last_movers < direct_events_below; }

    void reset()
    {
        *this = spkm_policy();
    }

    void observe(const spkm_policy_counters& c, double n, int tiles, int nr)
    {
        if (mov_pending_valid) { last_movers = (unsigned long long)c.movers; movers_known = true; }
        if (c.may_regroup && n >= 4096 && c.one_cluster_steps < 0.125 * std::ceil(n / 16.0) && c.ambig < 0.9 * n) regroup_wanted = true;
        if (!hint_pending && prune_pending_a == 0 && !skip_pending) crowded = c.ambig >= 0.9 * n;
        if (ev_latched && dual_latched && c.full_opened) { ev_calls = 0; ev_cum_movers = 0; }
        else if (ev_latched && mov_pending_valid) ev_cum_movers += (unsigned long long)c.movers;
        if (c.listed > 0.05 * n) exact_cooldown = 8;
        const bool short_list = (n - c.kept) <= 0.02 * n;
        const double bar = short_list ? (pt_next ? 1.5 : 2.5) : (pt_next ? 2.5 : 4.0);
        pt_next = skip_pending && c.kept >= 0.6 * n && (std::ceil(n / 16.0) - c.skipped) * 16.0 > bar * (n - c.kept);
        blocks_next = skip_pending && c.kept >= 0.9 * n && (std::ceil(n / 16.0) - c.skipped) * 16.0 <= 8.0 * (n - c.kept);
        const int a_prune = quad_split(nr);
        const int t = std::max(1, tiles);
        if (hint_pending) {
            const double steps = std::max(0.0, n / 16.0 - c.skipped - c.msteps) * t + c.pairs2;
            const double early = c.early + c.early2;
            const double share = steps > 0.0 ? early / steps : 1.0;
            const bool was_late = hint_late_pending;
            const double all_pairs = n / 16.0 * t;
            if (!was_late && share < 0.15 && steps > 0.25 * all_pairs && hint_late_left == 0) hint_late_left = 2;
            hint_late = hint_late_left > 0;
            const bool fallback_to_late = !was_late && hint_late && quad_split_late(nr) > quad_split(nr);
            const bool poor = early < 0.05 * steps && steps > 0.01 * n / 16.0;
            if (c.listed > 0.005 * n || (poor && !fallback_to_late)) {
                hint_fail_streak = std::min(hint_fail_streak + 1, 4);
                hint_cooldown = 1 << hint_fail_streak;
            } else if (poor) {
            } else {
                hint_fail_streak = 0;
                if (c.ambig <= 0.002 * n && prune_cooldown == 0 && a_prune < nr) prune_next_a = a_prune;
            }
        } else if (prune_pending_a == 0)
            prune_next_a = (c.ambig <= 0.002 * n && prune_cooldown == 0 && a_prune < nr) ? a_prune : 0;
        else if (c.listed > 0.005 * n) { prune_next_a = 0; prune_cooldown = 16; }
    }

    struct choice {
        bool exact;
        int prune_a;
        bool want_hint;
    };
    choice next(bool no_prune, bool no_hint, bool quad)
    {
        if (prune_cooldown > 0) prune_cooldown--;
        if (hint_cooldown > 0) hint_cooldown--;
        const bool cooling = exact_cooldown > 0;
        if (cooling) exact_cooldown--;
        choice ch;
        ch.exact = cooling;
        ch.prune_a = no_prune ? 0 : prune_next_a;
        ch.want_hint = ch.prune_a == 0 && !no_prune && !no_hint && hint_cooldown == 0 && quad && !crowded;
        return ch;
    }
    bool take_hinted_split(int nr, bool no_late_split)
    {
        const bool late = hint_late && quad_split_late(nr) > quad_split(nr) && !no_late_split;
        if (hint_late_left > 0) hint_late_left--;
        if (hint_late_left == 0) hint_late = false;
        return late;
    }
    void launched(int rounds_all, int rounds, bool hinted, bool hinted_late, bool skipping, bool movers_counted,
                  bool by_events = false, bool both_forms = false)
    {
        prune_pending_a = rounds_all < rounds ? rounds_all : 0;
        hint_pending = hinted;
        hint_late_pending = hinted && hinted_late;
        skip_pending = skipping;
        mov_pending_valid = movers_counted;
        ev_latched = by_events;
        dual_latched = by_events && both_forms;
    }
    bool few_movers(double n, bool pair_events = false) const
    {
        return !movers_known || (double)last_movers * (pair_events ? 2.0 : 3.0) <= n;
    }
    bool form_on_device() const { return !movers_known; }
    void sums_by_events() { ev_pending = true; ev_calls++; }
    void sums_by_full_pass() { ev_pending = false; ev_calls = 0; ev_cum_movers = 0; }
    bool refresh_due(double n) const { return ev_calls >= 256 || (double)ev_cum_movers > 8.0 * n; }
    static unsigned long long event_cap(unsigned long long n, bool pair_events = false) { return pair_events ? n / 2ull : 2ull * (n / 3ull); }
};

constexpr int SEG_POINTS = 2048, SEG_POINTS_MAX = 8192, SEG_EVENTS = 256, SEG_DENSE = 256;
inline int seg_points(long long n, int blocks)
{
    const long long want = n / ((long long)std::max(1, blocks) * 16);
    return (int)std::max<long long>(SEG_POINTS, std::min<long long>(SEG_POINTS_MAX, want));
}
constexpr int spkm_plan_kt = 32, spkm_plan_span = 16384, spkm_plan_span_pt = 4096, spkm_plan_seg = SEG_POINTS;
inline int spkm_wide_kt(long long p, size_t lds_max)
// ... 274 lines not shown
                        : 0xffffffffu;
    pl.reuse = pl.kept && in.sort_reusable;
    pl.nk_incr = pl.kept;
    pl.direct = pl.ev_path && !pl.dual && pol.events_direct() && !in.no_direct_events;
    pl.seg_ev = (pol.movers_known && pol.last_movers < 100000) ? SEG_EVENTS : spkm_plan_seg;
}
constexpr int spkm_movers = 32, spkm_mover_kmin = 64, spkm_mover_kmax = 1024;
SPKM_HD constexpr unsigned long long spkm_mover_key(float d, int k)
{
    const float v = d >= 0.f ? d : __builtin_inff();
    return ((unsigned long long)__builtin_bit_cast(unsigned, v) << 32) | (unsigned long long)(unsigned)(0x7fffffff - k);
}
SPKM_HD constexpr int spkm_mover_rank(const float* delta, int K, int k)
{
    const unsigned long long mine = spkm_mover_key(delta[k], k);
    int r = 0;
    for (int j = 0; j < K; j++) r += spkm_mover_key(delta[j], j) > mine ? 1 : 0;
    return r;
}
SPKM_HD constexpr float spkm_mover_dr(float d_next, float dmax)
{
    return (dmax >= 0.f && dmax < __builtin_inff() && d_next >= 0.f) ? d_next : __builtin_inff();
}
inline float spkm_pick_movers(const float* delta, int K, int* list, int* slot)
{
    float dmax = 0.f, dn = __builtin_inff();
    bool bad = false;
    for (int k = 0; k < K; k++) {
        const int r = spkm_mover_rank(delta, K, k);
        slot[k] = r < spkm_movers ? r : -1;
        if (r < spkm_movers) list[r] = k;
        if (r == spkm_movers) dn = delta[k];
        if (!(delta[k] >= 0.f)) bad = true; else dmax = std::max(dmax, delta[k]);
    }
    return spkm_mover_dr(dn, bad ? __builtin_inff() : dmax);
}
constexpr bool spkm_mover_default_on = true;
struct spkm_mover_plan {
    bool eligible = false, on = false;
    long long cap = 0;
    int tiles = 1, pl = 4, nr = 0;
};
inline spkm_mover_plan spkm_plan_movers(const spkm_call_in& in, const spkm_call_plan& pl, int K, int sw)
{
    spkm_mover_plan m;
    m.nr = pl.nr;
    m.eligible = in.quad && K >= spkm_mover_kmin && K <= spkm_mover_kmax && pl.drift && pl.skip_enabled && !pl.pt_mode &&
                 !pl.sp_on && pl.erode && !in.has_map;
    m.on = m.eligible && (sw > 0 || (sw == 0 && spkm_mover_default_on));
    m.cap = m.on ? pl.npad / 16 + 1 : 0;
    return m;
}
constexpr int spkm_movers2 = 64, spkm_mover2_kmin = 96;
inline void spkm_pick_movers2(const float* delta, int K, int* list, int* slot, float* dr)
{
    float dmax = 0.f, dn = __builtin_inff(), dn2 = __builtin_inff();
    bool bad = false;
    for (int k = 0; k < K; k++) {
        const int r = spkm_mover_rank(delta, K, k);
        slot[k] = r < spkm_movers2 ? r : -1;
        if (r < spkm_movers2) list[r] = k;
        if (r == spkm_movers) dn = delta[k];
        if (r == spkm_movers2 && K >= spkm_mover2_kmin) dn2 = delta[k];
        if (!(delta[k] >= 0.f)) bad = true; else dmax = std::max(dmax, delta[k]);
    }
    dr[0] = spkm_mover_dr(dn, bad ? __builtin_inff() : dmax);
    dr[1] = spkm_mover_dr(dn2, bad ? __builtin_inff() : dmax);
}
constexpr bool spkm_mover2_default_on = true;
struct spkm_mover2_plan {
    bool eligible = false, on = false;
    long long cap = 0;
    int tiles = 2, pl = 4, nr = 0;
};
inline spkm_mover2_plan spkm_plan_movers2(const spkm_mover_plan& first, const spkm_call_plan& pl, int K, int sw)
{
    spkm_mover2_plan m;
    m.nr = pl.nr;
    m.eligible = first.eligible && K >= spkm_mover2_kmin;
    m.on = m.eligible && first.on && (sw > 0 || (sw == 0 && spkm_mover2_default_on));
    m.cap = m.on ? pl.npad / 16 + 1 : 0;
    return m;
}
```

### sparsifiedkmeans_amd/csrc/screen.hip

```cpp
#include "common.h"
#include <hip/amd_detail/amd_hip_unsafe_atomics.h>

__global__ void k_prep_tiles_f32(const double* __restrict__ C, int p, int K, int G, double gamma,
                                 float* __restrict__ T32, unsigned long long* __restrict__ cmax_bits, int pl_last,
                                 int swz, double* __restrict__ Cs, double* __restrict__ keep,
                                 const int* __restrict__ mlist = nullptr, int mtiles = 1)
{
    if (Cs != nullptr || keep != nullptr) {
        const size_t pkk = (size_t)p * K;
        for (size_t t = (size_t)blockIdx.x * blockDim.x + threadIdx.x; t < pkk; t += (size_t)gridDim.x * blockDim.x) {
            if (keep != nullptr) keep[t] = C[t];
            if (Cs != nullptr) {
                const int k = (int)(t % K);
                const size_t r = t / K;
                double v = C[(size_t)k * p + r];
                if (gamma > 0.0) v = v / gamma;
                Cs[t] = v;
            }
        }
    }
    const size_t total = (size_t)(G + (mlist != nullptr ? mtiles : 0)) * (p + 1) * SCREEN_KT;
    double mx = 0.0;
    for (size_t t = (size_t)blockIdx.x * blockDim.x + threadIdx.x; t < total; t += (size_t)gridDim.x * blockDim.x) {
        int kk = (int)(t % SCREEN_KT);
// ... 872 lines not shown
{
    if (gate != nullptr && *gate == 0u) return;
    __shared__ unsigned long long s_pts;
    if (threadIdx.x == 0) s_pts = 0ull;
    __syncthreads();
    unsigned long long mine = 0ull;
    for (int k = threadIdx.x; k < K; k += blockDim.x) {
        const int fresh = (force || touched[k]) ? 1 : 0;
        const int nd = (fresh || !same[k]) ? 1 : 0;
        need[k] = nd;
        touched[k] = fresh;
        if (nd) mine += nk[k];
    }
    if (mine) atomicAdd(&s_pts, mine);
    __syncthreads();
    if (threadIdx.x == 0) {
        atomicAdd(reinterpret_cast<unsigned long long*>(counters + NL_EXACT_TOTAL), s_pts);
        counters[NL_EXACT_PTS] = (unsigned)(s_pts > 0xffffffffull ? 0xffffffffull : s_pts);
    }
}

__global__ __launch_bounds__(256) void k_cluster_restore(const int* __restrict__ need, int K, int p,
                                                         double* __restrict__ sums, double* __restrict__ counts,
                                                         double* __restrict__ cache_s, double* __restrict__ cache_c,
                                                         const unsigned* __restrict__ gate = nullptr)
{
    if (gate != nullptr && *gate == 0u) return;
    const size_t pk = (size_t)K * p;
    for (size_t t = (size_t)blockIdx.x * blockDim.x + threadIdx.x; t < pk; t += (size_t)gridDim.x * blockDim.x) {
        const int k = (int)(t / p);
        if (need[k]) { cache_s[t] = sums[t]; cache_c[t] = counts[t]; }
        else { sums[t] = cache_s[t]; counts[t] = cache_c[t]; }
    }
}

__global__ __launch_bounds__(256) void k_cluster_stats(const int* __restrict__ need, int K, const int* __restrict__ ibeg,
                                                       const int* __restrict__ icnt, const double* __restrict__ it_obj,
                                                       const double* __restrict__ it_max,
                                                       const long long* __restrict__ it_imax, double* __restrict__ cl_obj,
                                                       double* __restrict__ cl_max, long long* __restrict__ cl_imax,
                                                       double* __restrict__ stats)
{
    __shared__ double s_o[256], s_m[256];
    __shared__ long long s_i[256];
    const int tid = threadIdx.x;
    double o = 0.0, m = -1.0;
    long long im = 0x7fffffffffffffffLL;
    for (int k = tid; k < K; k += 256) {
        if (need[k]) {
            double ko = 0.0, km = -1.0;
            long long ki = 0x7fffffffffffffffLL;
            for (int t = ibeg[k]; t < ibeg[k] + icnt[k]; t++) {
                ko += it_obj[t];
                if (it_max[t] > km || (it_max[t] == km && it_imax[t] < ki)) { km = it_max[t]; ki = it_imax[t]; }
            }
            cl_obj[k] = ko; cl_max[k] = km; cl_imax[k] = ki;
        }
        o += cl_obj[k];
        if (cl_max[k] > m || (cl_max[k] == m && cl_imax[k] < im)) { m = cl_max[k]; im = cl_imax[k]; }
    }
    s_o[tid] = o; s_m[tid] = m; s_i[tid] = im;
    __syncthreads();
    for (int off = 128; off > 0; off >>= 1) {
        if (tid < off) {
            s_o[tid] += s_o[tid + off];
            if (s_m[tid + off] > s_m[tid] || (s_m[tid + off] == s_m[tid] && s_i[tid + off] < s_i[tid])) {
                s_m[tid] = s_m[tid + off];
                s_i[tid] = s_i[tid + off];
            }
        }
        __syncthreads();
    }
    if (tid == 0) { stats[0] = s_o[0]; stats[1] = s_m[0]; stats[2] = (double)s_i[0]; }
}
__global__ void k_pick_form(unsigned* __restrict__ counters, unsigned ev_cap, int* __restrict__ nitems)
{
    const bool full = counters[NL_EVENTS] > ev_cap;
    counters[NL_GATE_EVENTS] = full ? 0u : 1u;
    counters[NL_GATE_FULL] = full ? 1u : 0u;
    nitems[NI_FULL] = 0;
    nitems[NI_EVENTS] = 0;
    nitems[NI_PAIR_CHUNKS] = 0;
}

__global__ __launch_bounds__(256) void k_regroup_keys(const float* __restrict__ bnd, long long npad, long long n, int K,
                                                      const double* __restrict__ cum, int* __restrict__ keys)
{
    const double cum_now = *cum;
    for (long long i = (long long)blockIdx.x * blockDim.x + threadIdx.x; i < n; i += (long long)gridDim.x * blockDim.x) {
        const float ub = bnd[i];
        const double lb = (double)bnd[hb_lb(npad) + i] - cum_now;
        int a = reinterpret_cast<const int*>(bnd)[hb_assign(npad) + i];
        if ((unsigned)a >= (unsigned)K) a = 0;
        keys[i] = 2 * a + ((lb >= 1.5 * (double)ub) ? 0 : 1);
    }
}
__global__ __launch_bounds__(256) void k_regroup_apply(const int* __restrict__ perm, const int* __restrict__ oldmap,
                                                       int* __restrict__ newmap, const float* __restrict__ bnd_old,
                                                       float* __restrict__ bnd_new, long long npad, long long n)
{
    for (long long j = (long long)blockIdx.x * blockDim.x + threadIdx.x; j < npad; j += (long long)gridDim.x * blockDim.x) {
        if (j < n) {
            const int o = perm[j];
            newmap[j] = oldmap != nullptr ? oldmap[o] : o;
            bnd_new[j] = bnd_old[o];
            bnd_new[hb_lb(npad) + j] = bnd_old[hb_lb(npad) + o];
            bnd_new[hb_assign(npad) + j] = bnd_old[hb_assign(npad) + o];
        } else {
            bnd_new[j] = 0.f; bnd_new[hb_lb(npad) + j] = 0.f; bnd_new[hb_assign(npad) + j] = 0.f;
        }
    }
}

__global__ void k_fill_jc(long long* __restrict__ jc, long long n, long long s)
{
    for (long long i = (long long)blockIdx.x * blockDim.x + threadIdx.x; i <= n; i += (long long)gridDim.x * blockDim.x) jc[i] = i * s;
}

struct spkm_zero_jobs {
    unsigned* p[8];
    unsigned long long words[8];
    int n;
};
__global__ __launch_bounds__(256) void k_zero_many(const spkm_zero_jobs j)
{
    for (int q = 0; q < j.n; q++) {
        unsigned* d = j.p[q];
        for (unsigned long long i = (unsigned long long)blockIdx.x * blockDim.x + threadIdx.x; i < j.words[q];
             i += (unsigned long long)gridDim.x * blockDim.x)
            d[i] = 0u;
    }
}
__global__ void k_zero_u64_gated(unsigned long long* __restrict__ dst, int n, const unsigned* __restrict__ gate)
{
    if (gate != nullptr && *gate == 0u) return;
    const int i = blockIdx.x * blockDim.x + threadIdx.x;
    if (i < n) dst[i] = 0ull;
}

template <int PPT>
__global__ __launch_bounds__(256) void k_combine_screen(const float* __restrict__ scr_m1,
                                                        const float* __restrict__ scr_m2,
                                                        const int* __restrict__ scr_k, long long n, int G,
                                                        const float* __restrict__ xnr, int fixed_s,
                                                        const unsigned long long* __restrict__ cmax_bits,
                                                        int* __restrict__ assign, int* __restrict__ list,
                                                        unsigned int* __restrict__ nlist,
                                                        float* __restrict__ bnd, long long npad, int skipping,
                                                        const int* __restrict__ todo,
                                                        const double* __restrict__ cum, int lib_valid,
                                                        int* __restrict__ touched, int K,
                                                        unsigned long long* __restrict__ nk,
                                                        int lazy, int* __restrict__ ev_pt, int* __restrict__ ev_k,
                                                        unsigned long long* __restrict__ nk_ev, unsigned ev_cap,
                                                        unsigned* __restrict__ wgstat, int* __restrict__ ev_o = nullptr,
                                                        const int* __restrict__ map = nullptr, int trusted = 0)
{
    constexpr int EVCAP = 2048;
    static_assert(4 * 64 * PPT * 2 <= EVCAP, "the four waves' events of one trip must fit the empty stage");
    __shared__ int s_evp[EVCAP], s_evk[EVCAP];
    const bool pair = ev_o != nullptr;
    __shared__ unsigned s_evn, s_evbase, s_mov, s_over, s_valid, s_done;
    const double cum_now = cum ? *cum : 0.0;
    extern __shared__ __attribute__((aligned(16))) char smem_c[];
    int* delta = reinterpret_cast<int*>(smem_c);
    unsigned* evc = reinterpret_cast<unsigned*>(smem_c) + (nk ? K : 0);
// ... 1033 lines not shown
```

### sparsifiedkmeans_amd/csrc/screen_quad.hip

```cpp
#include "common.h"
#include "quad_steps.inc"
#include <type_traits>

#ifndef SPKM_SQ_IRBITS
#error "build with -DSPKM_SQ_IRBITS=16|32 -DSPKM_SQ_PTS=0|1 (csrc/build.sh)"
#endif

typedef float f2v __attribute__((ext_vector_type(2)));
typedef float f4v __attribute__((ext_vector_type(4)));

__device__ __forceinline__ float raw_min_f32(float a, float b)
{
    float r;
    asm("v_min_f32 %0, %1, %2" : "=v"(r) : "v"(a), "v"(b));
    return r;
}
__device__ __forceinline__ float raw_max_f32(float a, float b)
{
    float r;
    asm("v_max_f32 %0, %1, %2" : "=v"(r) : "v"(a), "v"(b));
    return r;
}
__device__ __forceinline__ int quad_min_i32(int v)
{
// ... 174 lines not shown
                            consider((k < K) ? v : __builtin_inff(), k);
                        }
                    }
                    if (PL == 5) {
                        const int k = extra_k0 + l4;
                        consider((k < K) ? acc4 : __builtin_inff(), k);
                    }
                }
                m1 = quad_min_f32(lo);
                const bool win = (lo == m1);
                seg = (unsigned)(__ballot(win) >> (ps * 4)) & 0xfu;
                first = seg ? __builtin_ctz(seg) : 0;
                m2 = quad_min_f32((l4 == first) ? hi : lo);
            };
            evaluate();
            int a_eff = A;
            if (A < NR && hint != nullptr) {
                const float hv = hraw;
                const bool fine = !(i < n) || m2 >= hint_c * hv * hv;
                if (!__all(fine)) {
                    SPKM_QUAD_ROUNDS(SPKM_GUARD_B)
                    evaluate();
                    a_eff = NR;
                } else
                    npruned++;
            }
            float full = m1;
            if (a_eff < NR) {
                const int kwin = quad_min_i32((l4 == first && seg != 0u) ? klo : 0x7fffffff);
                const bool is_extra = PL == 5 && kwin >= extra_k0;
                const int cpiece = ((kwin - k0) >> 2) << 4, celem = ((kwin - k0) & 3) << 2;
                const int ebase = extra_base + (kwin - extra_k0) * 4;
                float accb = 0.f;
#define SPKM_QUAD_FINISH(r, EXTRA)                                                                          \
    if constexpr (NR > r && r >= A) {                                                                       \
        const bool okr = (r < NR - 1) || l4 < nvl;                                                          \
        const int t4 = o##r << 4;                                                                           \
        const int adr = (EXTRA && is_extra) ? ((t4 >> 7) << 4) + ebase : (t4 ^ cpiece) + celem;             \
        const float cv = *reinterpret_cast<const float*>(smem + adr);                                       \
        const float tv = okr ? cv + x##r : 0.f;                                                             \
        accb = __builtin_fmaf(tv, tv, accb);                                                                \
    }
#define SPKM_QUAD_FINISH_ALL(EXTRA)                                                                         \
    SPKM_QUAD_FINISH(0, EXTRA) SPKM_QUAD_FINISH(1, EXTRA) SPKM_QUAD_FINISH(2, EXTRA) SPKM_QUAD_FINISH(3, EXTRA)     \
    SPKM_QUAD_FINISH(4, EXTRA) SPKM_QUAD_FINISH(5, EXTRA) SPKM_QUAD_FINISH(6, EXTRA) SPKM_QUAD_FINISH(7, EXTRA)     \
    SPKM_QUAD_FINISH(8, EXTRA) SPKM_QUAD_FINISH(9, EXTRA) SPKM_QUAD_FINISH(10, EXTRA) SPKM_QUAD_FINISH(11, EXTRA)   \
    SPKM_QUAD_FINISH(12, EXTRA) SPKM_QUAD_FINISH(13, EXTRA) SPKM_QUAD_FINISH(14, EXTRA) SPKM_QUAD_FINISH(15, EXTRA)
                if (PL == 5 && __any(is_extra)) { SPKM_QUAD_FINISH_ALL(true) } else { SPKM_QUAD_FINISH_ALL(false) }
#undef SPKM_QUAD_FINISH_ALL
#undef SPKM_QUAD_FINISH
#undef SPKM_QUAD_ROUNDS
#undef SPKM_QUAD_ROUND_G
#undef SPKM_GUARD_A
#undef SPKM_GUARD_B
                full = m1 + quad_sum_f32(kwin == 0x7fffffff ? 0.f : accb);
            }
            if (l4 == first && i < n) {
                const bool none = seg == 0u;
                const int at = PTS ? vbase + ps : i;
                m1o[at] = none ? __builtin_inff() : full;
                m2o[at] = none ? __builtin_inff() : m2;
                ko[at] = none ? -1 : klo;
            }
            };
            if constexpr (PL0 == 5) {
                if (rot > 0 && (t / R) % rot != bm.tile) evaluate_step(std::integral_constant<int, 4>{});
                else evaluate_step(std::integral_constant<int, 5>{});
            } else
                evaluate_step(std::integral_constant<int, PL0>{});
        }
    }
    if (counters != nullptr && lane == 0 && npruned) atomicAdd(ticket + 1, npruned);
}

template <int NR, typename IR, int TWO, bool PTS>
__global__ __launch_bounds__(1024) void k_screen_quad(
    const IR* __restrict__ ir, const float* __restrict__ xval, const float* __restrict__ T32, int p, int n, int fixed_s,
    int K, const spkm_blockmap* __restrict__ bmap, int chunk_points, float* __restrict__ scr_m1,
    float* __restrict__ scr_m2, int* __restrict__ scr_k, int extra_tile,
    const float* __restrict__ hint, float hint_c, unsigned* __restrict__ counters, const int* __restrict__ todo,
    int todo_points,
    const char* __restrict__ rec, int rec_R,
    const int* __restrict__ recmap,
    int todo_slot)
{
    extern __shared__ __attribute__((aligned(16))) char smem[];
    const spkm_blockmap bm = bmap[blockIdx.x];
    if (bm.tile < 0) return;
    if (todo != nullptr && counters[todo_slot] == 0u) return;
    const int tid = threadIdx.x;
    const int pl = (bm.pad >> 16) & 0xff;
    const size_t tile_bytes = (size_t)(p + 1) * SCREEN_KT * 4;
    const size_t extra_bytes = pl == 5 ? (size_t)(p + 1) * 16 : 0;
    {
        const float4* src = reinterpret_cast<const float4*>(T32 + (size_t)bm.tile * (p + 1) * SCREEN_KT);
        float4* dst = reinterpret_cast<float4*>(smem);
        for (size_t t = tid; t < tile_bytes / 16; t += blockDim.x) dst[t] = src[t];
        if (pl == 5) {
            const float4* esrc = reinterpret_cast<const float4*>(T32 + (size_t)extra_tile * (p + 1) * SCREEN_KT);
            float4* edst = reinterpret_cast<float4*>(smem + tile_bytes);
            for (size_t t = tid; t < extra_bytes / 16; t += blockDim.x) edst[t] = esrc[t];
        }
    }
    unsigned* ticket = reinterpret_cast<unsigned*>(smem + tile_bytes + extra_bytes);
    if (tid == 0) { ticket[0] = 0u; ticket[1] = 0u; }
    __syncthreads();
    float* m1o = scr_m1 + (size_t)bm.tile * n;
    float* m2o = scr_m2 + (size_t)bm.tile * n;
    int* ko = scr_k + (size_t)bm.tile * n;
    const int eb = (int)tile_bytes, ek = extra_tile * SCREEN_KT;
    constexpr int A = TWO == 0 ? NR : (TWO == 2 && quad_split_late(NR, PTS) > 0 ? quad_split_late(NR, PTS) : quad_split(NR, PTS));
    int nv = n, chunk_v = chunk_points, tp = 0;
    if (todo != nullptr) {
        if (PTS) { tp = (int)counters[todo_slot]; nv = (tp + 15) & ~15; }
        else nv = (int)counters[todo_slot] * 16;
        chunk_v = max(256, min(chunk_points, (nv / (int)(gridDim.x * 2)) & ~255));
    }
    if (pl == 4) screen_quad_body<NR, IR, 4, A, PTS>(ir, xval, p, n, nv, fixed_s, K, bm, chunk_v, m1o, m2o, ko, smem, ticket, eb, ek, hint, hint_c, counters, todo, tp, rec, rec_R, recmap);
    else if (pl == 5) screen_quad_body<NR, IR, 5, A, PTS>(ir, xval, p, n, nv, fixed_s, K, bm, chunk_v, m1o, m2o, ko, smem, ticket, eb, ek, hint, hint_c, counters, todo, tp, rec, rec_R, recmap);
    else if (pl == 2) screen_quad_body<NR, IR, 2, A, PTS>(ir, xval, p, n, nv, fixed_s, K, bm, chunk_v, m1o, m2o, ko, smem, ticket, eb, ek, hint, hint_c, counters, todo, tp, rec, rec_R, recmap);
    else screen_quad_body<NR, IR, 1, A, PTS>(ir, xval, p, n, nv, fixed_s, K, bm, chunk_v, m1o, m2o, ko, smem, ticket, eb, ek, hint, hint_c, counters, todo, tp, rec, rec_R, recmap);
    if (counters != nullptr) {
        __syncthreads();
        if (tid == 0 && ticket[1]) atomicAdd(counters + (todo_slot == NL_TODO_M ? NL_MEARLY : NL_EARLY), ticket[1]);
    }
}


#if SPKM_SQ_IRBITS == 16
typedef unsigned short sq_ir_t;
#else
typedef unsigned int sq_ir_t;
#endif
#define SPKM_SQ_CAT2(a, b, c) a##b##_##c
#define SPKM_SQ_CAT(a, b, c) SPKM_SQ_CAT2(a, b, c)

const void* SPKM_SQ_CAT(spkm_sq_kernel_, SPKM_SQ_IRBITS, SPKM_SQ_PTS)(int rounds, int a_rounds)
{
    constexpr bool PTS = SPKM_SQ_PTS != 0;
    typedef sq_ir_t IR;
    const bool late = a_rounds < rounds && quad_split_late(rounds, PTS) > 0 && a_rounds == quad_split_late(rounds, PTS);
    const bool two = a_rounds < rounds;
    switch (rounds) {
#define SPKM_QUAD_CASE(N)                                                                                   \
    case N:                                                                                                 \
        if (late) return (const void*)k_screen_quad<N, IR, (quad_split_late(N, PTS) > 0 ? 2 : 0), PTS>;     \
        return two && quad_split(N, PTS) < N ? (const void*)k_screen_quad<N, IR, (quad_split(N, PTS) < N ? 1 : 0), PTS> : (const void*)k_screen_quad<N, IR, 0, PTS>;
        SPKM_QUAD_CASE(1) SPKM_QUAD_CASE(2) SPKM_QUAD_CASE(3) SPKM_QUAD_CASE(4) SPKM_QUAD_CASE(5) SPKM_QUAD_CASE(6)
        SPKM_QUAD_CASE(7) SPKM_QUAD_CASE(8) SPKM_QUAD_CASE(9) SPKM_QUAD_CASE(10) SPKM_QUAD_CASE(11) SPKM_QUAD_CASE(12)
        SPKM_QUAD_CASE(13) SPKM_QUAD_CASE(14) SPKM_QUAD_CASE(15) SPKM_QUAD_CASE(16)
#undef SPKM_QUAD_CASE
    default: return nullptr;
    }
}
```

### sparsifiedkmeans_amd/csrc/update.hip

```cpp
#include "common.h"
#include <hip/amd_detail/amd_hip_unsafe_atomics.h>

__global__ void k_prep_tiles(const double* __restrict__ C, int p, int K, int KT, int G, double gamma,
                             double* __restrict__ negCt)
{
    const size_t total = (size_t)G * (p + 1) * KT;
    for (size_t t = (size_t)blockIdx.x * blockDim.x + threadIdx.x; t < total; t += (size_t)gridDim.x * blockDim.x) {
        const int kk = (int)(t % KT);
        const size_t rest = t / KT;
        const int r = (int)(rest % (p + 1));
        const int g = (int)(rest / (p + 1));
        const int k = g * KT + kk;
        double v = 0.0;
        if (r < p && k < K) {
            v = C[(size_t)k * p + r];
            if (gamma > 0.0) v = v / gamma;
            v = -v;
        }
        negCt[t] = v;
    }
}

__global__ __launch_bounds__(256) void k_combine(const double* __restrict__ part_acc,
                                                 const int* __restrict__ part_k, long long n, int G, int K,
// ... 827 lines not shown
            int re;
            if (rec != nullptr) {
                const char* b = rec + (size_t)i * (size_t)R;
                xe = reinterpret_cast<const double*>(b)[j];
                re = (int)reinterpret_cast<const IR*>(b + (size_t)s * 8)[j];
            } else { xe = x[i * s + j]; re = (int)ir[i * s + j]; }
            unsafeAtomicAdd(&sums[(size_t)k * p + re], sign * xe);
            unsafeAtomicAdd(&counts[(size_t)k * p + re], sign);
            if ((unsigned)kold < (unsigned)K) {
                unsafeAtomicAdd(&sums[(size_t)kold * p + re], -xe);
                unsafeAtomicAdd(&counts[(size_t)kold * p + re], -1.0);
            }
        }
    }
}

__global__ __launch_bounds__(256) void k_finalize_centers(const double* __restrict__ sums,
                                                          const double* __restrict__ counts,
                                                          const double* __restrict__ nk_f64, int p, int K,
                                                          double gamma, double* __restrict__ centers,
                                                          double* __restrict__ blk_dff2, unsigned* __restrict__ ticket,
                                                          double* __restrict__ out, const double* __restrict__ obj2,
                                                          double* __restrict__ host_res = nullptr, unsigned long long seq = 0ull)
{
    __shared__ double s_part[4];
    __shared__ unsigned s_last;
    const size_t total = (size_t)p * K;
    double acc = 0.0;
    for (size_t t = (size_t)blockIdx.x * blockDim.x + threadIdx.x; t < total; t += (size_t)gridDim.x * blockDim.x) {
        const int k = (int)(t / p);
        const double oldv = centers[t];
        double newv = oldv;
        if (nk_f64[k] > 0.0) newv = (gamma * sums[t]) / (counts[t] + 1e-16);
        centers[t] = newv;
        const double d = oldv - newv;
        acc += d * d;
    }
    for (int off = 32; off > 0; off >>= 1) acc += __shfl_down(acc, off);
    if ((threadIdx.x & 63) == 0) s_part[threadIdx.x >> 6] = acc;
    __syncthreads();
    if (threadIdx.x == 0) {
        double o = 0.0;
        for (int w = 0; w < (int)(blockDim.x >> 6); w++) o += s_part[w];
        blk_dff2[blockIdx.x] = o;
        __threadfence();
        s_last = atomicAdd(ticket, 1u) == gridDim.x - 1 ? 1u : 0u;
    }
    __syncthreads();
    if (!s_last || threadIdx.x >= 64) return;
    __threadfence();
    double o = 0.0;
    for (int b = threadIdx.x; b < (int)gridDim.x; b += 64) o += __builtin_nontemporal_load(blk_dff2 + b);
    for (int off = 32; off > 0; off >>= 1) o += __shfl_down(o, off);
    if (threadIdx.x == 0) {
        out[0] = o;
        if (obj2) out[1] = *obj2;
        *ticket = 0u;
    }
    if (host_res != nullptr) {
        for (int k = threadIdx.x; k < K; k += 64) host_res[3 + k] = nk_f64[k];
        if (threadIdx.x == 0) {
            host_res[1] = o;
            host_res[2] = obj2 ? *obj2 : __longlong_as_double(0x7ff8000000000000LL);
        }
        __threadfence_system();
        if (threadIdx.x == 0)
            __hip_atomic_store(reinterpret_cast<unsigned long long*>(host_res), seq, __ATOMIC_RELEASE, __HIP_MEMORY_SCOPE_SYSTEM);
    }
}

__global__ void k_nk_to_f64(const unsigned long long* __restrict__ nk, int K, double* __restrict__ out)
{
    const int k = blockIdx.x * blockDim.x + threadIdx.x;
    if (k < K) out[k] = (double)nk[k];
}

__global__ void k_call_tail(const unsigned long long* __restrict__ nk, int K, double* __restrict__ nk_f,
                            const double* __restrict__ stats, double* __restrict__ obj2, double* __restrict__ d_stats,
                            unsigned long long* __restrict__ d_nk, const unsigned* __restrict__ bstat, int bstat_n,
                            unsigned* __restrict__ counters, int lazy = 0, double* __restrict__ cache_s = nullptr,
                            const double* __restrict__ cache_c = nullptr, size_t pk = 0, double* __restrict__ sums = nullptr,
                            double* __restrict__ counts = nullptr, unsigned* __restrict__ host_out = nullptr, unsigned seq = 0u,
                            unsigned long long work_steps = 0ull, int work_tiles = 0, int work_nr = 0, int work_a = 0,
                            int work_flags = 0, unsigned long long screen_n = 0ull, int mover_on = 0)
{
    if (screen_n > 0ull && blockIdx.x == 0 && threadIdx.x == 0) {
        unsigned long long v = screen_n;
        if (work_flags & 2) v = (work_flags & 4) ? (unsigned long long)counters[NL_TODO] : (unsigned long long)counters[NL_TODO] * 16ull;
        if (mover_on) v += (unsigned long long)counters[NL_MCERT] * 16ull;
        if (mover_on & 2) v += (unsigned long long)counters[NL_MCERT2] * 16ull;
        if (v > screen_n) v = screen_n;
        counters[NL_SCREENED] = (unsigned)v;
        *reinterpret_cast<unsigned long long*>(counters + NL_SCREENED_TOTAL) += v;
    }
    if (work_tiles > 0 && blockIdx.x == 0 && threadIdx.x == 0) {
        unsigned long long steps = work_steps;
        if (work_flags & 2) steps = (work_flags & 4) ? ((unsigned long long)counters[NL_TODO] + 15ull) / 16ull : (unsigned long long)counters[NL_TODO];
        unsigned long long r = steps * (unsigned long long)work_tiles * (unsigned long long)((work_flags & 1) ? work_a : work_nr);
        if (!(work_flags & 1) && work_a < work_nr) {
            const unsigned long long saved = (unsigned long long)counters[NL_EARLY] * (unsigned long long)(work_nr - work_a);
            r -= saved < r ? saved : r;
        }
        if (mover_on) {
            unsigned long long rm = (unsigned long long)counters[NL_TODO_M] * (unsigned long long)((work_flags & 1) ? work_a : work_nr);
            if (!(work_flags & 1) && work_a < work_nr) {
                const unsigned long long saved = (unsigned long long)counters[NL_MEARLY] * (unsigned long long)(work_nr - work_a);
                rm -= saved < rm ? saved : rm;
            }
            r += rm;
        }
        if (mover_on & 2) {
            unsigned long long rm = (unsigned long long)counters[NL_TODO_M2] * 2ull * (unsigned long long)((work_flags & 1) ? work_a : work_nr);
            if (!(work_flags & 1) && work_a < work_nr) {
                const unsigned long long saved = (unsigned long long)counters[NL_MEARLY2] * (unsigned long long)(work_nr - work_a);
                rm -= saved < rm ? saved : rm;
            }
            r += rm;
        }
        *reinterpret_cast<unsigned long long*>(counters + NL_ROUNDS_DONE) += r;
        *reinterpret_cast<unsigned long long*>(counters + NL_ROUNDS_FULL) += work_steps * (unsigned long long)work_tiles * (unsigned long long)work_nr;
    }
    if (cache_s != nullptr) {
        for (size_t t = (size_t)blockIdx.x * blockDim.x + threadIdx.x; t < pk; t += (size_t)gridDim.x * blockDim.x) {
            const double c = cache_c[t];
            double v = cache_s[t];
            if (c == 0.0 && v != 0.0) { v = 0.0; cache_s[t] = 0.0; }
            sums[t] = v;
            counts[t] = c;
        }
    }
    if (blockIdx.x == 0 && bstat_n > 0) {
        __shared__ unsigned s_k[256], s_s[256];
        unsigned a = 0, b = 0;
        for (int t = threadIdx.x; t < bstat_n; t += blockDim.x) { a += bstat[BS_STRIDE * t + BS_KEPT]; b += bstat[BS_STRIDE * t + BS_SKIPPED]; }
        s_k[threadIdx.x] = a; s_s[threadIdx.x] = b;
        __syncthreads();
        for (int off = 128; off > 0; off >>= 1) {
            if ((int)threadIdx.x < off) { s_k[threadIdx.x] += s_k[threadIdx.x + off]; s_s[threadIdx.x] += s_s[threadIdx.x + off]; }
            __syncthreads();
        }
        if (threadIdx.x == 0) {
            counters[NL_KEPT] += s_k[0];
            counters[NL_SKIPPED] += s_s[0];
            *reinterpret_cast<unsigned long long*>(counters + NL_SKIPPED_TOTAL) += (unsigned long long)s_s[0];
        }
    }
    if (host_out != nullptr && blockIdx.x == 0 && threadIdx.x == 0) {
        for (int j = 0; j < SPKM_REPORT_WORDS; j++) host_out[j] = counters[j];
        __hip_atomic_store(host_out + SPKM_REPORT_WORDS, seq, __ATOMIC_RELEASE, __HIP_MEMORY_SCOPE_SYSTEM);
    }
    const int k = blockIdx.x * blockDim.x + threadIdx.x;
    if (k < K) {
        const unsigned long long v = nk[k];
        nk_f[k] = (double)v;
        if (d_nk) d_nk[k] = v;
    }
    const double nan = __longlong_as_double(0x7ff8000000000000LL);
    if (k == 0) *obj2 = lazy ? nan : stats[0];
    if (k < 3 && d_stats) d_stats[k] = lazy ? nan : stats[k];
}

template __global__ void k_accumulate_atomic<unsigned short>(const long long*, const unsigned short*, const double*,
    const int*, int, long long, double*, double*);
template __global__ void k_accumulate_atomic<unsigned int>(const long long*, const unsigned int*, const double*,
    const int*, int, long long, double*, double*);
template __global__ void k_accumulate_sorted<unsigned short>(const long long*, const unsigned short*, const double*,
    const int*, const long long*, const int4*, const int*, int, int, double*, double*);
template __global__ void k_accumulate_sorted<unsigned int>(const long long*, const unsigned int*, const double*,
    const int*, const long long*, const int4*, const int*, int, int, double*, double*);
template __global__ void k_accumulate_sliced<unsigned short>(const long long*, const unsigned short*, const double*,
    const int*, const long long*, const int4*, const int*, int, int, int, int, double*, double*);
template __global__ void k_accumulate_sliced<unsigned int>(const long long*, const unsigned int*, const double*,
    const int*, const long long*, const int4*, const int*, int, int, int, int, double*, double*);
```

### sparsifiedkmeans_amd/engine.py

```python
from __future__ import annotations

import ctypes as C
import time
import warnings

import numpy as np
import torch

from . import _lib
from .ops import Context


def _p(t: torch.Tensor):
    return C.c_void_p(t.data_ptr())


class Shard:

    def __init__(self, ctx: Context, handle, keep=()):
        self.ctx = ctx
        self.handle = handle
        self._keep = keep
        p, n, nnz, bits = C.c_uint64(), C.c_uint64(), C.c_uint64(), C.c_int()
        _lib.check(_lib.lib().spkm_shard_info(handle, C.byref(p), C.byref(n), C.byref(nnz), C.byref(bits)))
# ... 242 lines not shown
    def allreduce_step(self):
        if comm_size(self.ctx) > 0:
            _lib.check(_lib.lib().spkm_allreduce_f64_dev(self.ctx.handle, _p(self.reduce), self.reduce.numel()),
                       "spkm_allreduce_f64_dev")
            return
        from .distributed import allreduce_

        allreduce_(self.reduce, self.group)

    def finalize_step(self, centers: torch.Tensor):
        _lib.check(_lib.lib().spkm_finalize_dev(self.ctx.handle, self.p, self.K, _p(self.reduce), self.gamma,
                                                _p(centers), _p(self.out)), "spkm_finalize_dev")

    def assign_accumulate_step(self, centers: torch.Tensor, want_mind: bool = True):
        assert centers.dtype == torch.float64 and centers.is_contiguous() and tuple(centers.shape) == (self.K, self.p)
        g = self.gamma if self.unbiased else 0.0
        _lib.check(_lib.lib().spkm_assign_accumulate_dev(self.ctx.handle, self.shard.handle, self.K, _p(centers), g,
                                                         _p(self.assign), _p(self.mind) if want_mind else None,
                                                         _p(self.stats), _p(self.nk), _p(self.reduce)),
                   "spkm_assign_accumulate_dev")

    def distances(self, centers_used: torch.Tensor) -> torch.Tensor:
        assert centers_used.dtype == torch.float64 and centers_used.is_contiguous() and tuple(centers_used.shape) == (self.K, self.p)
        g = self.gamma if self.unbiased else 0.0
        _lib.check(_lib.lib().spkm_distances_stats_dev(self.ctx.handle, self.shard.handle, self.K, _p(centers_used), g,
                                                       _p(self.assign), _p(self.mind), _p(self.stats)),
                   "spkm_distances_stats_dev")
        return self.mind

    def last_path_info(self) -> tuple[int, int]:
        a = (C.c_int64 * 2)()
        _lib.check(_lib.lib().spkm_last_path_info(self.ctx.handle, a))
        return int(a[0]), int(a[1])

    def exact_pass_points(self) -> tuple[int, int]:
        a = (C.c_int64 * 2)()
        _lib.check(_lib.lib().spkm_exact_pass_points(self.ctx.handle, a))
        return int(a[0]), int(a[1])

    def screen_work_totals(self) -> tuple[int, int]:
        a = (C.c_int64 * 2)()
        _lib.check(_lib.lib().spkm_screen_work_totals(self.ctx.handle, a))
        return int(a[0]), int(a[1])

    def last_screen_rounds(self) -> tuple[int, int]:
        a = (C.c_int64 * 2)()
        _lib.check(_lib.lib().spkm_last_screen_rounds(self.ctx.handle, a))
        return int(a[0]), int(a[1])

    def last_screen_mode(self) -> tuple[int, ...]:
        a = (C.c_int64 * 8)()
        _lib.check(_lib.lib().spkm_last_screen_mode(self.ctx.handle, a))
        return tuple(int(v) for v in a)

    def last_events_form(self) -> tuple[int, int]:
        a = (C.c_int64 * 2)()
        _lib.check(_lib.lib().spkm_last_events_form(self.ctx.handle, a))
        return int(a[0]), int(a[1])

    def last_assign_tile(self) -> tuple[int, ...]:
        a = (C.c_int64 * 6)()
        _lib.check(_lib.lib().spkm_last_assign_tile(self.ctx.handle, a))
        return tuple(int(v) for v in a)

    def last_screen_tile(self) -> tuple[int, int]:
        a = (C.c_int64 * 2)()
        _lib.check(_lib.lib().spkm_last_screen_tile(self.ctx.handle, a))
        return int(a[0]), int(a[1])

    def last_screen_points(self) -> tuple[int, int]:
        a = (C.c_int64 * 2)()
        _lib.check(_lib.lib().spkm_last_screen_points(self.ctx.handle, a))
        return int(a[0]), int(a[1])

    def last_mover_steps(self) -> tuple[int, int, int]:
        a = (C.c_uint64 * 3)()
        _lib.check(_lib.lib().spkm_last_mover_steps(self.ctx.handle, a))
        return int(a[0]), int(a[1]), int(a[2])

    def last_mover_steps2(self) -> tuple[int, int, int]:
        a = (C.c_uint64 * 3)()
        _lib.check(_lib.lib().spkm_last_mover_steps2(self.ctx.handle, a))
        return int(a[0]), int(a[1]), int(a[2])

    def iterate(self, centers: torch.Tensor, want_mind: bool = True):
        from .distributed import is_distributed

        if is_distributed() and comm_size(self.ctx) == 0:
            self.assign_accumulate_step(centers, want_mind)
            self.allreduce_step()
            self.finalize_step(centers)
            return self.out
        assert centers.dtype == torch.float64 and centers.is_contiguous() and tuple(centers.shape) == (self.K, self.p)
        _lib.check(_lib.lib().spkm_lloyd_iter(self.ctx.handle, self.shard.handle, self.K, _p(centers), self.gamma,
                                              1 if self.unbiased else 0, _p(self.assign),
                                              _p(self.mind) if want_mind else None, _p(self.stats),
                                              _p(self.nk), _p(self.reduce), _p(self.out)), "spkm_lloyd_iter")
        return self.out

    def iterate_host(self, centers: torch.Tensor, want_mind: bool = True) -> np.ndarray:
        from .distributed import is_distributed

        if is_distributed() and comm_size(self.ctx) == 0:
            self.iterate(centers, want_mind)
            pk = self.p * self.K
            return torch.cat([self.out, self.reduce[2 * pk: 2 * pk + self.K]]).cpu().numpy()
        assert centers.dtype == torch.float64 and centers.is_contiguous() and tuple(centers.shape) == (self.K, self.p)
        if self._host_res is None or self._host_res.size != 2 + self.K:
            self._host_res = np.zeros(2 + self.K, np.float64)
        _lib.check(_lib.lib().spkm_lloyd_iter_host(self.ctx.handle, self.shard.handle, self.K, _p(centers), self.gamma,
                                                   1 if self.unbiased else 0, _p(self.assign),
                                                   _p(self.mind) if want_mind else None, _p(self.stats),
                                                   _p(self.nk), _p(self.reduce), _p(self.out),
                                                   self._host_res.ctypes.data), "spkm_lloyd_iter_host")
        return self._host_res.copy()

    def global_nk(self) -> torch.Tensor:
        pk = self.p * self.K
        return self.reduce[2 * pk: 2 * pk + self.K]

    def last_assign_kernel_ms(self) -> float:
        ms = C.c_double()
        _lib.check(_lib.lib().spkm_last_assign_kernel_ms(self.ctx.handle, C.byref(ms)))
        return ms.value


def fwht_device(ctx: Context, x: torch.Tensor) -> torch.Tensor:
    assert x.dtype == torch.float64 and x.is_contiguous() and x.dim() == 2
    y = torch.empty_like(x)
    _lib.check(_lib.lib().spkm_fwht_dev(ctx.handle, x.shape[1], x.shape[0], _p(x), _p(y)), "spkm_fwht_dev")
    return y


def mix_device(ctx: Context, x: torch.Tensor, p2: int, sign: torch.Tensor | None, premul: float,
               postdiv: float) -> torch.Tensor:
    assert x.dtype == torch.float64 and x.is_contiguous() and x.dim() == 2
    n, p = x.shape
    y = torch.empty((n, p2), dtype=torch.float64, device=x.device)
    _lib.check(_lib.lib().spkm_mix_dev(ctx.handle, p, p2, n, _p(x), _p(sign) if sign is not None else None,
                                       float(premul), float(postdiv), _p(y)), "spkm_mix_dev")
    return y


def mix_sample_device(ctx: Context, x: torch.Tensor, p2: int, sign: torch.Tensor | None, premul: float,
                      postdiv: float, s: int, seed: int, col0: int, ir_out: torch.Tensor, x_out: torch.Tensor):
    assert x.dtype == torch.float64 and x.is_contiguous() and x.dim() == 2
    n, p = x.shape
    assert ir_out.numel() >= n * s and x_out.numel() >= n * s and x_out.dtype == torch.float64
    bits = ir_out.element_size() * 8
    _lib.check(_lib.lib().spkm_mix_sample_dev(ctx.handle, p, p2, n, _p(x), _p(sign) if sign is not None else None,
                                              float(premul), float(postdiv), int(s), int(seed) & (2**64 - 1),
                                              int(col0), _p(ir_out), bits, _p(x_out)), "spkm_mix_sample_dev")


def record_bytes(s: int, ir_bits: int = 16) -> int:
    return int(_lib.lib().spkm_record_bytes(int(s), int(ir_bits)))


def mix_sample_records_device(ctx: Context, x: torch.Tensor, p2: int, sign: torch.Tensor | None, premul: float,
                              postdiv: float, s: int, seed: int, col0: int, rec_out: torch.Tensor, ir_bits: int = 16):
    assert x.dtype == torch.float64 and x.is_contiguous() and x.dim() == 2
    n, p = x.shape
    assert rec_out.dtype == torch.uint8 and rec_out.is_contiguous() and rec_out.numel() >= n * record_bytes(s, ir_bits)
    _lib.check(_lib.lib().spkm_mix_sample_rec_dev(ctx.handle, p, p2, n, _p(x), _p(sign) if sign is not None else None,
                                                  float(premul), float(postdiv), int(s), int(seed) & (2**64 - 1),
                                                  int(col0), int(ir_bits), _p(rec_out)), "spkm_mix_sample_rec_dev")
# ... 441 lines not shown
```

Before: 283.3.

## Add cold-start pilot screen that derives per-block hints and gates the plain screen

On an unhinted first call with large n, a pilot screen runs on one 16-point sample per 1024-point block. A new kernel turns the pilot's best and second distances into a per-block pruning hint and counts coherent blocks. If enough blocks are coherent, a device-side gate runs a hinted, narrower screen and skips the full plain screen. Otherwise the plain screen runs as before. This aims to cut screening work on cold calls, at the cost of extra launches and pilot work, and it also relaxes some policy latches when the hint was used.

```diff
diff --git a/include/spkm.h b/include/spkm.h
--- a/include/spkm.h
+++ b/include/spkm.h
@@ -96,6 +96,7 @@
 int spkm_last_screen_points(spkm_ctx *ctx, int64_t info[2]);
 int spkm_last_mover_steps(spkm_ctx *ctx, uint64_t out[3]);
 int spkm_last_mover_steps2(spkm_ctx *ctx, uint64_t out[3]);
+int spkm_last_cold_hint(spkm_ctx *ctx, uint64_t out[4]);
 
 int spkm_exact_pass_points(spkm_ctx *ctx, int64_t info[2]);
 int spkm_screen_work_totals(spkm_ctx *ctx, int64_t info[2]);
diff --git a/sparsifiedkmeans_amd/_lib.py b/sparsifiedkmeans_amd/_lib.py
--- a/sparsifiedkmeans_amd/_lib.py
+++ b/sparsifiedkmeans_amd/_lib.py
@@ -139,6 +139,7 @@
     L.spkm_last_screen_points.argtypes = [_vp, C.POINTER(C.c_int64)]
     L.spkm_last_mover_steps.argtypes = [_vp, C.POINTER(C.c_uint64)]
     L.spkm_last_mover_steps2.argtypes = [_vp, C.POINTER(C.c_uint64)]
+    L.spkm_last_cold_hint.argtypes = [_vp, C.POINTER(C.c_uint64)]
     L.spkm_dense_assign_dev.argtypes = [_vp, _u64, _u64, _vp, _u64, _vp, _vp, _vp]
     L.spkm_dense_accumulate_dev.argtypes = [_vp, _u64, _u64, _vp, _u64, _vp, _vp, _vp]
     L.spkm_dense_assign_src_dev.argtypes = [_vp, _u64, _u64, C.c_int, _vp, _u64, _vp, _vp, _vp]
diff --git a/sparsifiedkmeans_amd/csrc/api.hip b/sparsifiedkmeans_amd/csrc/api.hip
--- a/sparsifiedkmeans_amd/csrc/api.hip
+++ b/sparsifiedkmeans_amd/csrc/api.hip
@@ -33,6 +33,7 @@
     w.force_point_list = on("SPKM_FORCE_POINT_LIST");
     w.mover_tile = on("SPKM_NO_MOVER_TILE") ? -1 : (on("SPKM_MOVER_TILE") ? 1 : 0);
     w.mover_tile2 = on("SPKM_NO_MOVER_TILE2") ? -1 : (on("SPKM_MOVER_TILE2") ? 1 : 0);
+    w.cold_hint = on("SPKM_NO_COLD_HINT") ? -1 : (on("SPKM_COLD_HINT") ? 1 : 0);
     w.wide_screen = on("SPKM_WIDE_SCREEN");
     w.wide_bounds = on("SPKM_WIDE_BOUNDS");
     w.far_screen = on("SPKM_FAR_SCREEN");
@@ -144,7 +145,7 @@
     devbuf* all[] = {&ctx->tiles, &ctx->part_acc, &ctx->part_k, &ctx->blk_obj, &ctx->blk_max, &ctx->blk_imax,
                      &ctx->nk, &ctx->stats, &ctx->perm, &ctx->offs, &ctx->cursor, &ctx->items, &ctx->nitems,
                      &ctx->bmap, &ctx->blk_dff, &ctx->ct, &ctx->tmp_assign, &ctx->tmp_mind, &ctx->mscr, &ctx->dbg, &ctx->t32, &ctx->scr_m1, &ctx->scr_m2,
-                     &ctx->scr_k, &ctx->cmax, &ctx->list, &ctx->nlist, &ctx->dn_x, &ctx->dn_c, &ctx->dn_nk, &ctx->bmapq, &ctx->bmapm, &ctx->bmapm2, &ctx->todo, &ctx->todo_m, &ctx->todo_m2, &ctx->bstat, &ctx->nk_ev, &ctx->fin_ticket, &ctx->wgstat, &ctx->offs2, &ctx->cursor2, &ctx->hist2,
+                     &ctx->scr_k, &ctx->cmax, &ctx->list, &ctx->nlist, &ctx->dn_x, &ctx->dn_c, &ctx->dn_nk, &ctx->bmapq, &ctx->bmapm, &ctx->bmapm2, &ctx->todo, &ctx->todo_m, &ctx->todo_m2, &ctx->todo_p, &ctx->bstat, &ctx->nk_ev, &ctx->fin_ticket, &ctx->wgstat, &ctx->offs2, &ctx->cursor2, &ctx->hist2,
                      &ctx->items2, &ctx->perm_o, &ctx->mix_scr};
     for (devbuf* b : all) release(*b);
     if (ctx->h_res) (void)hipHostFree(ctx->h_res);
diff --git a/sparsifiedkmeans_amd/csrc/api_internal.h b/sparsifiedkmeans_amd/csrc/api_internal.h
--- a/sparsifiedkmeans_amd/csrc/api_internal.h
+++ b/sparsifiedkmeans_amd/csrc/api_internal.h
@@ -58,6 +58,7 @@
     bool sliced_sums = false;
     int x_slab_rows = 0;
     bool force_point_list = false;
+    int cold_hint = 0;
     int mover_tile2 = 0;
     int mover_tile = 0;
 };
@@ -76,6 +77,7 @@
     bool direct_events = false;
     bool pair_events = false;
     bool sums_only = false;
+    bool cold = false;
     bool movers2 = false;
     bool movers = false;
     bool dual = false;
@@ -88,7 +90,7 @@
     size_t lds_max = 0;
     size_t mem_bytes = 0;
     devbuf tiles, part_acc, part_k, blk_obj, blk_max, blk_imax, nk, stats, perm, offs, cursor, items, nitems,
-        bmap, blk_dff, ct, tmp_assign, tmp_mind, mscr, dbg, t32, scr_m1, scr_m2, scr_k, cmax, list, nlist, dn_x, dn_c, dn_nk, bmapq, bmapm, bmapm2, todo, todo_m, todo_m2, bstat, nk_ev, fin_ticket, wgstat, offs2, cursor2, hist2, items2, perm_o;
+        bmap, blk_dff, ct, tmp_assign, tmp_mind, mscr, dbg, t32, scr_m1, scr_m2, scr_k, cmax, list, nlist, dn_x, dn_c, dn_nk, bmapq, bmapm, bmapm2, todo, todo_m, todo_m2, todo_p, bstat, nk_ev, fin_ticket, wgstat, offs2, cursor2, hist2, items2, perm_o;
     devbuf mix_scr;
     double* h_res = nullptr;
     double* h_res_dev = nullptr;
diff --git a/sparsifiedkmeans_amd/csrc/api_lloyd.hip b/sparsifiedkmeans_amd/csrc/api_lloyd.hip
--- a/sparsifiedkmeans_amd/csrc/api_lloyd.hip
+++ b/sparsifiedkmeans_amd/csrc/api_lloyd.hip
@@ -887,6 +887,22 @@
     return SPKM_OK;
 }
 
+extern "C" int spkm_last_cold_hint(spkm_ctx* ctx, uint64_t out[4])
+{
+    if (!ctx || !out) return SPKM_ERR_NULL_ARG;
+    out[0] = out[1] = out[2] = out[3] = 0;
+    if (ctx->last.path == 1 && ctx->last.cold && ctx->nlist.p) {
+        HIP_TRY(hipSetDevice(ctx->device));
+        HIP_TRY(hipStreamSynchronize(ctx->stream));
+        unsigned v[SPKM_REPORT_WORDS] = {0};
+        HIP_TRY(hipMemcpy(v, ctx->nlist.p, sizeof(v), hipMemcpyDeviceToHost));
+        out[0] = v[NL_TODO_P]; out[1] = v[NL_COLD_COHERENT];
+        out[2] = v[NL_GATE_HINT] ? 2 : 1;
+        out[3] = v[NL_GATE_HINT] ? v[NL_EARLY] : 0;
+    }
+    return SPKM_OK;
+}
+
 extern "C" int spkm_last_screen_rounds(spkm_ctx* ctx, int64_t info[2])
 {
     if (!ctx || !info) return SPKM_ERR_NULL_ARG;
diff --git a/sparsifiedkmeans_amd/csrc/api_lloyd_fused.inc b/sparsifiedkmeans_amd/csrc/api_lloyd_fused.inc
--- a/sparsifiedkmeans_amd/csrc/api_lloyd_fused.inc
+++ b/sparsifiedkmeans_amd/csrc/api_lloyd_fused.inc
@@ -71,6 +71,7 @@
     spkm_call_plan pl;
     spkm_mover_plan mv;
     spkm_mover2_plan mv2;
+    spkm_cold_plan cold;
     spkm_screen_report rep;
     spkm_zero_jobs zj;
     int kt = SCREEN_KT;
@@ -212,7 +213,8 @@
             if ((rc = ensure(ctx, ctx->nk_ev, (size_t)2 * K * 8))) return rc;
             zero_later(ctx->nk_ev.p, (size_t)2 * K * 8);
         }
-        if (pl.hinted) {
+        if (cold.on && (rc = ensure(ctx, ctx->todo_p, (size_t)cold.blocks * 4))) return rc;
+        if (pl.hinted || cold.on) {
             rep.hint_late = pl.late;
             if (sm->hintu_len < pl.npad) {
                 HIP_TRY(regrow(sm->hintu, (size_t)pl.npad * 4));
@@ -334,15 +336,43 @@
         int a_recR = sm->rec_R, a_tp = pl.pt_mode ? 1 : 0;
         const int* a_recmap = sm->map;
         int a_slot = NL_TODO;
+        const unsigned *a_gate = nullptr, *a_nogate = nullptr;
         void* args[] = {&a_ir, &a_xf, &a_t, &a_p, &a_n, &a_s, &a_K, &a_bm, &a_chunk, &a_m1, &a_m2, &a_k, &a_extra,
-                        &a_hint, &a_hc, &a_cnt, &a_todo, &a_tp, &a_rec, &a_recR, &a_recmap, &a_slot};
+                        &a_hint, &a_hc, &a_cnt, &a_todo, &a_tp, &a_rec, &a_recR, &a_recmap, &a_slot, &a_gate};
+        if (cold.on) {
+            hipLaunchKernelGGL(k_pilot_list, dim3((unsigned)std::min<long long>((cold.blocks + 255) / 256, 256)), dim3(256), 0, ctx->stream,
+                               (int*)ctx->todo_p.p, (int)cold.blocks, a_cnt);
+            const int* p_todo = (const int*)ctx->todo_p.p;
+            const float* p_hint = nullptr;
+            int p_slot = NL_TODO_P;
+            void* pargs[] = {&a_ir, &a_xf, &a_t, &a_p, &a_n, &a_s, &a_K, &a_bm, &a_chunk, &a_m1, &a_m2, &a_k, &a_extra,
+                             &p_hint, &a_hc, &a_cnt, &p_todo, &a_tp, &a_rec, &a_recR, &a_recmap, &p_slot, &a_nogate};
+            HIP_TRY(hipLaunchKernel(kern, dim3(ctx->bmapq_blocks), dim3(1024), pargs, lds, ctx->stream));
+            HIP_TRY(hipGetLastError());
+            hipLaunchKernelGGL(k_pilot_hints, dim3((unsigned)std::min<long long>((cold.blocks + 15) / 16, 1024)), dim3(256), 0, ctx->stream,
+                               (const float*)a_m1, (const float*)a_m2, a_n, pl.npad, pl.Gs, (int)cold.blocks, sm->hintu, a_cnt);
+            HIP_TRY(hipGetLastError());
+            const void* kern_h = screen_quad_kernel<IR>(pl.nr, cold.a, false);
+            HIP_TRY(allow_lds(ctx, kern_h, lds));
+            const float* h_hint = sm->hintu;
+            const int* h_todo = nullptr;
+            int h_chunk = (int)std::min<long long>(pl.chunk, ctx->sw.x_hint_chunk >= 256 ? ctx->sw.x_hint_chunk : 256);
+            { int c2 = 256; while (c2 * 2 <= h_chunk) c2 *= 2; h_chunk = c2; }
+            const unsigned* h_gate = a_cnt + NL_GATE_HINT;
+            void* hargs[] = {&a_ir, &a_xf, &a_t, &a_p, &a_n, &a_s, &a_K, &a_bm, &h_chunk, &a_m1, &a_m2, &a_k, &a_extra,
+                             &h_hint, &a_hc, &a_cnt, &h_todo, &a_tp, &a_rec, &a_recR, &a_recmap, &a_slot, &h_gate};
+            HIP_TRY(hipLaunchKernel(kern_h, dim3(ctx->bmapq_blocks), dim3(1024), hargs, lds, ctx->stream));
+            HIP_TRY(hipGetLastError());
+            a_gate = a_cnt + NL_GATE_PLAIN;
+        }
+        rep.cold = cold.on;
         if (mv.on) {
             const float* m_t = a_t + (size_t)pl.G * (p + 1) * SCREEN_KT;
             const spkm_blockmap* m_bm = (const spkm_blockmap*)ctx->bmapm.p;
             const int* m_todo = (const int*)ctx->todo_m.p;
             int m_K = SPKM_MOVERS, m_extra = 0, m_slot = NL_TODO_M;
             void* margs[] = {&a_ir, &a_xf, &m_t, &a_p, &a_n, &a_s, &m_K, &m_bm, &a_chunk, &a_m1, &a_m2, &a_k, &m_extra,
-                             &a_hint, &a_hc, &a_cnt, &m_todo, &a_tp, &a_rec, &a_recR, &a_recmap, &m_slot};
+                             &a_hint, &a_hc, &a_cnt, &m_todo, &a_tp, &a_rec, &a_recR, &a_recmap, &m_slot, &a_nogate};
             HIP_TRY(hipLaunchKernel(kern, dim3(ctx->bmapm_blocks), dim3(1024), margs, lds, ctx->stream));
             HIP_TRY(hipGetLastError());
             const int* m2_todo = (const int*)ctx->todo_m2.p;
@@ -350,7 +380,7 @@
                 const spkm_blockmap* m2_bm = (const spkm_blockmap*)ctx->bmapm2.p;
                 int m2_K = SPKM_MOVERS2, m2_slot = NL_TODO_M2;
                 void* m2args[] = {&a_ir, &a_xf, &m_t, &a_p, &a_n, &a_s, &m2_K, &m2_bm, &a_chunk, &a_m1, &a_m2, &a_k, &m_extra,
-                                  &a_hint, &a_hc, &a_cnt, &m2_todo, &a_tp, &a_rec, &a_recR, &a_recmap, &m2_slot};
+                                  &a_hint, &a_hc, &a_cnt, &m2_todo, &a_tp, &a_rec, &a_recR, &a_recmap, &m2_slot, &a_nogate};
                 HIP_TRY(hipLaunchKernel(kern, dim3(ctx->bmapm2_blocks), dim3(1024), m2args, lds, ctx->stream));
                 HIP_TRY(hipGetLastError());
             }
@@ -783,7 +813,7 @@
                            ev ? (const double*)(sm->cl_cache + cc_counts(pk)) : (const double*)nullptr, ev ? pk : (size_t)0,
                            ev ? sums : (double*)nullptr, ev ? counts : (double*)nullptr,
                            sm->nlist_pending ? (unsigned*)nullptr : sm->h_nlist_dev, sm->nlist_seq + 1u,
-                           work_steps, work_tiles, pl.nr, rep.rounds_all, work_flags, (unsigned long long)n, (mv.on ? 1 : 0) | (mv2.on ? 2 : 0));
+                           work_steps, work_tiles, pl.nr, rep.rounds_all, work_flags, (unsigned long long)n, (mv.on ? 1 : 0) | (mv2.on ? 2 : 0), cold.on ? cold.a : 0);
         HIP_TRY(hipGetLastError());
         if (carry) {
             sm->hb_K = K; sm->hb_gamma = gamma; sm->hb_valid = true;
@@ -818,6 +848,7 @@
     spkm_plan_call(c.pl, c, c.sm->pol);
     c.mv = spkm_plan_movers(c, c.pl, K, ctx->sw.mover_tile);
     c.mv2 = spkm_plan_movers2(c.mv, c.pl, K, ctx->sw.mover_tile2);
+    c.cold = spkm_plan_cold_hint(c, c.pl, false, ctx->sw.force_form, ctx->sw.cold_hint);
     if ((rc = c.resources()) || (rc = c.mover_resources()) || (rc = c.bounds()) || (rc = c.screen<IR>())) return rc;
     const int ev = c.pl.ev_possible ? 2 : 1, max_items_ev_all = ev == 2 ? (int)((2 * c.n) / SEG_EVENTS) + 2 * K + 1 : 0;
     if ((rc = ensure(ctx, ctx->perm, (size_t)ev * c.n * 4)) || (rc = ensure(ctx, ctx->offs, (size_t)(ev * K + 1) * 8)) ||
@@ -892,6 +923,7 @@
         c.pairs2 = 2.0 * ((double)h[NL_MCERT2] + (double)h[NL_MSENT2]);
         c.early2 = h[NL_MEARLY2];
         c.full_opened = h[NL_GATE_FULL] != 0u;
+        c.cold_hinted = h[NL_GATE_HINT] != 0u;
         c.one_cluster_steps = h[NL_ONE_CLUSTER];
         c.may_regroup = sm->pend_full && sm->lazy && !sm->regroup_done;
         const int kt_seen = std::max(8, screen_tile_kt(ctx, s));
diff --git a/sparsifiedkmeans_amd/csrc/layout.h b/sparsifiedkmeans_amd/csrc/layout.h
--- a/sparsifiedkmeans_amd/csrc/layout.h
+++ b/sparsifiedkmeans_amd/csrc/layout.h
@@ -16,7 +16,9 @@
     NL_KEPT = 12,
     NL_EXACT_PTS = 13,
     NL_MOVERS = 14,
+    NL_COLD_TICKET = 15,
     NL_EVENTS = 16,
+    NL_COLD_COHERENT = 17,
     NL_GATE_EVENTS = 18,
     NL_GATE_FULL = 19,
     NL_CHECK_DIFF = 20,
@@ -27,6 +29,9 @@
     NL_MCERT2 = 25,
     NL_MSENT2 = 26,
     NL_MEARLY2 = 27,
+    NL_TODO_P = 28,
+    NL_GATE_HINT = 29,
+    NL_GATE_PLAIN = 30,
     NL_PER_CALL_END = 32,
     NL_EXACT_TOTAL = 32,
     NL_ROUNDS_DONE = 34,
@@ -35,8 +40,8 @@
     NL_SCREENED = 40,
     NL_WORDS = 64
 };
-constexpr int SPKM_REPORT_WORDS = 28;
-constexpr int SPKM_REPORT_BUF_WORDS = 32;
+constexpr int SPKM_REPORT_WORDS = 31;
+constexpr int SPKM_REPORT_BUF_WORDS = 40;
 constexpr int NL_ZERO_A = 0, NL_ZERO_A_END = NL_SKIPPED_TOTAL;
 constexpr int NL_ZERO_B = NL_SKIPPED_TOTAL + 2, NL_ZERO_B_END = NL_PER_CALL_END;
 
@@ -54,6 +59,9 @@
 static_assert(nl_reported(NL_MSTEPS2) && nl_reported(NL_MCERT2) && nl_reported(NL_MSENT2) && nl_reported(NL_MEARLY2) && nl_zeroed(NL_MSTEPS2) &&
               nl_zeroed(NL_TODO_M2) && nl_zeroed(NL_MCERT2) && nl_zeroed(NL_MSENT2) && nl_zeroed(NL_MEARLY2),
               "... and so are the second level's");
+static_assert(nl_reported(NL_TODO_P) && nl_reported(NL_COLD_COHERENT) && nl_reported(NL_GATE_HINT) && nl_reported(NL_GATE_PLAIN) &&
+              nl_zeroed(NL_TODO_P) && nl_zeroed(NL_COLD_COHERENT) && nl_zeroed(NL_COLD_TICKET) && nl_zeroed(NL_GATE_HINT) && nl_zeroed(NL_GATE_PLAIN),
+              "the first call's pilot: per-call words of the report, both gates closed at the top of a call");
 static_assert(nl_total_ok(NL_SKIPPED_TOTAL) && nl_total_ok(NL_EXACT_TOTAL) && nl_total_ok(NL_ROUNDS_DONE) &&
               nl_total_ok(NL_ROUNDS_FULL) && nl_total_ok(NL_SCREENED_TOTAL),
               "a running total is an aligned 64-bit pair that the per-call zeroing leaves alone");
diff --git a/sparsifiedkmeans_amd/csrc/policy.h b/sparsifiedkmeans_amd/csrc/policy.h
--- a/sparsifiedkmeans_amd/csrc/policy.h
+++ b/sparsifiedkmeans_amd/csrc/policy.h
@@ -24,6 +24,7 @@
     bool full_opened = false;
     double one_cluster_steps = 0;
     bool may_regroup = false;
+    bool cold_hinted = false;
 };
 
 struct spkm_policy {
@@ -63,10 +64,10 @@
     {
         if (mov_pending_valid) { last_movers = (unsigned long long)c.movers; movers_known = true; }
         if (c.may_regroup && n >= 4096 && c.one_cluster_steps < 0.125 * std::ceil(n / 16.0) && c.ambig < 0.9 * n) regroup_wanted = true;
-        if (!hint_pending && prune_pending_a == 0 && !skip_pending) crowded = c.ambig >= 0.9 * n;
+        if (!hint_pending && prune_pending_a == 0 && !skip_pending) crowded = c.cold_hinted ? false : c.ambig >= 0.9 * n;
         if (ev_latched && dual_latched && c.full_opened) { ev_calls = 0; ev_cum_movers = 0; }
         else if (ev_latched && mov_pending_valid) ev_cum_movers += (unsigned long long)c.movers;
-        if (c.listed > 0.05 * n) exact_cooldown = 8;
+        if (c.listed > 0.05 * n && !c.cold_hinted) exact_cooldown = 8;
         const bool short_list = (n - c.kept) <= 0.02 * n;
         const double bar = short_list ? (pt_next ? 1.5 : 2.5) : (pt_next ? 2.5 : 4.0);
         pt_next = skip_pending && c.kept >= 0.6 * n && (std::ceil(n / 16.0) - c.skipped) * 16.0 > bar * (n - c.kept);
@@ -507,3 +508,37 @@
     m.cap = m.on ? pl.npad / 16 + 1 : 0;
     return m;
 }
+constexpr int spkm_cold_block = 1024, spkm_cold_pilot = 16;
+SPKM_HD constexpr float spkm_cold_block_hint2(const float* m1, const float* r, int npts)
+{
+    float mx = 0.f, mn = __builtin_inff();
+    bool ok = npts > 0;
+    for (int j = 0; j < npts; j++) {
+        ok = ok && m1[j] >= 0.f && m1[j] < __builtin_inff() && r[j] < __builtin_inff() && r[j] >= 2.25f * m1[j];
+        mx = m1[j] > mx ? m1[j] : mx;
+        mn = m1[j] < mn ? m1[j] : mn;
+    }
+    return (ok && mx <= 2.25f * mn) ? mx : __builtin_inff();
+}
+constexpr unsigned spkm_cold_gate_num = 15, spkm_cold_gate_den = 100;
+SPKM_HD constexpr bool spkm_cold_gate_open(unsigned long long coherent, unsigned long long blocks)
+{
+    return blocks > 0 && coherent * spkm_cold_gate_den >= blocks * spkm_cold_gate_num;
+}
+constexpr long long spkm_cold_min_n = 4ll << 20;
+constexpr bool spkm_cold_default_on = true;
+struct spkm_cold_plan {
+    bool eligible = false, on = false;
+    int a = 0;
+    long long blocks = 0;
+};
+inline spkm_cold_plan spkm_plan_cold_hint(const spkm_call_in& in, const spkm_call_plan& pl, bool exact, int force_form, int sw)
+{
+    spkm_cold_plan c;
+    c.a = quad_split(pl.nr);
+    c.blocks = (in.n + spkm_cold_block - 1) / spkm_cold_block;
+    c.eligible = in.quad && in.fixed_s > 0 && !pl.bounds_ok && !pl.skip_enabled && !pl.pt_mode && !pl.hinted && pl.prune_a == 0 &&
+                 pl.Gs >= 2 && c.a < pl.nr && !exact && force_form == 0 && in.n > 0 && (in.n >= spkm_cold_min_n || sw > 0);
+    c.on = c.eligible && (sw > 0 || (sw == 0 && spkm_cold_default_on));
+    return c;
+}
diff --git a/sparsifiedkmeans_amd/csrc/screen.hip b/sparsifiedkmeans_amd/csrc/screen.hip
--- a/sparsifiedkmeans_amd/csrc/screen.hip
+++ b/sparsifiedkmeans_amd/csrc/screen.hip
@@ -978,6 +978,69 @@
     nitems[NI_EVENTS] = 0;
     nitems[NI_PAIR_CHUNKS] = 0;
 }
+__global__ void k_pilot_list(int* __restrict__ todo_p, int blocks, unsigned* __restrict__ counters)
+{
+    for (int b = blockIdx.x * blockDim.x + threadIdx.x; b < blocks; b += gridDim.x * blockDim.x) todo_p[b] = b * (spkm_cold_block / 16);
+    if (blockIdx.x == 0 && threadIdx.x == 0) counters[NL_TODO_P] = (unsigned)blocks;
+}
+__global__ __launch_bounds__(256) void k_pilot_hints(const float* __restrict__ m1p, const float* __restrict__ m2p, int n, long long npad,
+                                                     int tiles, int blocks, float* __restrict__ hint, unsigned* __restrict__ counters)
+{
+    __shared__ unsigned s_coh;
+    if (threadIdx.x == 0) s_coh = 0u;
+    __syncthreads();
+    const int lane = threadIdx.x & 63, sub = lane & 15, grp = lane >> 4;
+    const long long wave = ((long long)blockIdx.x * blockDim.x + threadIdx.x) >> 6, nwaves = ((long long)gridDim.x * blockDim.x) >> 6;
+    const float inf = __builtin_inff();
+    unsigned ncoh = 0;
+    for (long long b0 = wave * 4; b0 < blocks; b0 += nwaves * 4) {
+        const long long b = b0 + grp, i = b * spkm_cold_block + sub;
+        const bool live = b < blocks && i < n;
+        float best = inf, second = inf;
+        bool bad = false;
+        if (live)
+            for (int t = 0; t < tiles; t++) {
+                const float a = m1p[(size_t)t * n + i], c = m2p[(size_t)t * n + i];
+                bad = bad || !(a >= 0.f && a < inf) || !(c >= 0.f);
+                if (a < best) { second = fminf(second, best); best = a; }
+                else second = fminf(second, a);
+                second = fminf(second, c);
+            }
+        int ok = !live || (!bad && best < inf && second < inf && second >= 2.25f * best);
+        float mx = live ? best : 0.f, mn = live ? best : inf;
+#pragma unroll
+        for (int off = 8; off > 0; off >>= 1) {
+            ok &= __shfl_xor(ok, off);
+            mx = fmaxf(mx, __shfl_xor(mx, off));
+            mn = fminf(mn, __shfl_xor(mn, off));
+        }
+        const bool coherent = b < blocks && ok && mx <= 2.25f * mn;
+        const float hv = coherent ? sqrtf(mx) : inf;
+        if (b < blocks) {
+            if (sub == 0 && coherent) ncoh++;
+            const float4 h4 = make_float4(hv, hv, hv, hv);
+#pragma unroll 4
+            for (int j = 0; j < spkm_cold_block / 64; j++) {
+                const long long at = b * spkm_cold_block + j * 64 + sub * 4;
+                if (at < npad) *reinterpret_cast<float4*>(hint + at) = h4;
+            }
+        }
+    }
+    if (ncoh) atomicAdd(&s_coh, ncoh);
+    __syncthreads();
+    if (threadIdx.x == 0) {
+        if (s_coh) atomicAdd(counters + NL_COLD_COHERENT, s_coh);
+        __threadfence();
+        const unsigned tk = atomicAdd(counters + NL_COLD_TICKET, 1u);
+        if (tk == gridDim.x - 1) {
+            __threadfence();
+            const unsigned coh = atomicAdd(counters + NL_COLD_COHERENT, 0u);
+            const bool open = spkm_cold_gate_open(coh, (unsigned long long)blocks);
+            counters[NL_GATE_HINT] = open ? 1u : 0u;
+            counters[NL_GATE_PLAIN] = open ? 0u : 1u;
+        }
+    }
+}
 
 __global__ __launch_bounds__(256) void k_regroup_keys(const float* __restrict__ bnd, long long npad, long long n, int K,
                                                       const double* __restrict__ cum, int* __restrict__ keys)
diff --git a/sparsifiedkmeans_amd/csrc/screen_quad.hip b/sparsifiedkmeans_amd/csrc/screen_quad.hip
--- a/sparsifiedkmeans_amd/csrc/screen_quad.hip
+++ b/sparsifiedkmeans_amd/csrc/screen_quad.hip
@@ -280,12 +280,14 @@
     int todo_points,
     const char* __restrict__ rec, int rec_R,
     const int* __restrict__ recmap,
-    int todo_slot)
+    int todo_slot,
+    const unsigned* __restrict__ gate)
 {
     extern __shared__ __attribute__((aligned(16))) char smem[];
     const spkm_blockmap bm = bmap[blockIdx.x];
     if (bm.tile < 0) return;
     if (todo != nullptr && counters[todo_slot] == 0u) return;
+    if (gate != nullptr && *gate == 0u) return;
     const int tid = threadIdx.x;
     const int pl = (bm.pad >> 16) & 0xff;
     const size_t tile_bytes = (size_t)(p + 1) * SCREEN_KT * 4;
diff --git a/sparsifiedkmeans_amd/csrc/update.hip b/sparsifiedkmeans_amd/csrc/update.hip
--- a/sparsifiedkmeans_amd/csrc/update.hip
+++ b/sparsifiedkmeans_amd/csrc/update.hip
@@ -933,7 +933,7 @@
                             const double* __restrict__ cache_c = nullptr, size_t pk = 0, double* __restrict__ sums = nullptr,
                             double* __restrict__ counts = nullptr, unsigned* __restrict__ host_out = nullptr, unsigned seq = 0u,
                             unsigned long long work_steps = 0ull, int work_tiles = 0, int work_nr = 0, int work_a = 0,
-                            int work_flags = 0, unsigned long long screen_n = 0ull, int mover_on = 0)
+                            int work_flags = 0, unsigned long long screen_n = 0ull, int mover_on = 0, int cold_a = 0)
 {
     if (screen_n > 0ull && blockIdx.x == 0 && threadIdx.x == 0) {
         unsigned long long v = screen_n;
@@ -951,6 +951,13 @@
         if (!(work_flags & 1) && work_a < work_nr) {
             const unsigned long long saved = (unsigned long long)counters[NL_EARLY] * (unsigned long long)(work_nr - work_a);
             r -= saved < r ? saved : r;
+        }
+        if (cold_a > 0) {
+            r += (unsigned long long)counters[NL_TODO_P] * (unsigned long long)work_tiles * (unsigned long long)work_nr;
+            if (counters[NL_GATE_HINT] != 0u && cold_a < work_nr) {
+                const unsigned long long saved = (unsigned long long)counters[NL_EARLY] * (unsigned long long)(work_nr - cold_a);
+                r -= saved < r ? saved : r;
+            }
         }
         if (mover_on) {
             unsigned long long rm = (unsigned long long)counters[NL_TODO_M] * (unsigned long long)((work_flags & 1) ? work_a : work_nr);
diff --git a/sparsifiedkmeans_amd/engine.py b/sparsifiedkmeans_amd/engine.py
--- a/sparsifiedkmeans_amd/engine.py
+++ b/sparsifiedkmeans_amd/engine.py
@@ -348,6 +348,11 @@
         a = (C.c_uint64 * 3)()
         _lib.check(_lib.lib().spkm_last_mover_steps2(self.ctx.handle, a))
         return int(a[0]), int(a[1]), int(a[2])
+
+    def last_cold_hint(self) -> tuple[int, int, int, int]:
+        a = (C.c_uint64 * 4)()
+        _lib.check(_lib.lib().spkm_last_cold_hint(self.ctx.handle, a))
+        return int(a[0]), int(a[1]), int(a[2]), int(a[3])
 
     def iterate(self, centers: torch.Tensor, want_mind: bool = True):
         from .distributed import is_distributed
```

After: 287.0 (median of 6 runs). No clear change (+1.3%).
